# hzxie/Stereo-3D-Reconstruction

Hardware: AMD Instinct MI355X
Metric: stereo pairs/s forward (batch 32, 224x224 -> 32^3 voxel) (higher is better)
Workload: dtype f32

## Files before the change

include/s3r.h:

```cpp
#ifndef S3R_H
#define S3R_H

#include <stddef.h>
#include <stdint.h>

#ifdef __cplusplus
extern "C" {
#endif

#define S3R_ABI_VERSION 8

typedef enum s3r_status {
    S3R_OK = 0,
    S3R_ERR_INVALID = -1,
    S3R_ERR_HIP = -2,
    S3R_ERR_WORKSPACE = -3
} s3r_status;

typedef enum s3r_op {
    S3R_OP_CONV = 0,
    S3R_OP_DECONV = 1,
    S3R_OP_LINEAR = 2
} s3r_op;

typedef enum s3r_dtype {
    S3R_F32 = 0,
    S3R_BF16 = 1
} s3r_dtype;

typedef enum s3r_act { S3R_ACT_NONE = 0, S3R_ACT_RELU = 1, S3R_ACT_SIGMOID = 2,
                       S3R_ACT_LEAKY_RELU = 3, S3R_ACT_ELU = 4, S3R_ACT_TANH = 5  } s3r_act;

typedef enum s3r_layout { S3R_LAYOUT_PLAIN = 0, S3R_LAYOUT_WINO_H = 2, S3R_LAYOUT_WINO_DH = 3, S3R_LAYOUT_WINO_HW = 4,
                          S3R_LAYOUT_WINO_3D = 5, S3R_LAYOUT_DIFF = 6 } s3r_layout;

typedef enum s3r_algo { S3R_ALGO_AUTO = 0, S3R_ALGO_DIRECT = 1, S3R_ALGO_WINOGRAD = 2 } s3r_algo;

typedef struct s3r_conv_desc {
    int32_t op;
    int32_t ndim;
    int32_t batch;
    int32_t cin, cout;
    int32_t in_size;
    int32_t k, stride, pad;
    int32_t act;
    int32_t tag;
    int32_t tile;
    int32_t in_halo;
    int32_t out_halo;
    int32_t ksplit;
    int32_t dtype;
    int32_t in_layout;
    int32_t out_layout;
    int32_t algo;
    int32_t dilation;
    int32_t out_pad;
    float act_param;
} s3r_conv_desc;

typedef struct s3r_layer {
    s3r_conv_desc desc;
    const void* packed_w;
    const float* scale;
    const float* shift;
} s3r_layer;

int s3r_abi_version(void);
const char* s3r_last_error(void);

int s3r_conv_out_size(const s3r_conv_desc* d);
int s3r_conv_packed_elems(const s3r_conv_desc* d, int64_t* elems);
int s3r_conv_pack_weights(const s3r_conv_desc* d, const float* w, void* packed, void* stream);
int64_t s3r_conv_scratch_elems(const s3r_conv_desc* d);
int s3r_conv_forward(const s3r_conv_desc* d, const void* x, const void* packed_w, const float* scale,
                     const float* shift, void* y, float* scratch, int64_t scratch_elems, void* stream);

int64_t s3r_chain_workspace_elems(const s3r_layer* layers, int n_layers);
int s3r_chain_forward(const s3r_layer* layers, int n_layers, const void* x, void* y, float* ws, int64_t ws_elems,
                      int ws_fresh, void* stream);

int s3r_encoder_forward(const s3r_layer* layers, int n_layers, const float* images_left, const float* images_right,
                        void* features, float* ws, int64_t ws_elems, int ws_fresh, void* stream);
int s3r_decoder_forward(const s3r_layer* layers, int n_layers, const void* volume, float* occupancy, float* ws,
                        int64_t ws_elems, int ws_fresh, void* stream);

int s3r_encoder_forward_u8(const s3r_layer* layers, int n_layers, const uint8_t* images_left, const uint8_t* images_right,
                           void* features, float* ws, int64_t ws_elems, int ws_fresh, void* stream);

int s3r_channels_last_to_f32(const void* x, float* y, int batch, int channels, int64_t positions, void* stream);

int s3r_cost_volume_forward(const float* feat_left, const float* feat_right, float* volume, int batch, int channels,
                            int max_disp, int height, int width, int out_halo, void* stream);

int s3r_cost_volume_forward_wino(const float* feat_left, const float* feat_right, float* planes, int batch, int channels,
                                 int max_disp, int height, int width, void* stream);
int64_t s3r_conv_wino_input_elems(const s3r_conv_desc* d);
int s3r_conv_wino_input_layout(const s3r_conv_desc* d);
int s3r_cost_volume_forward_wino2(const float* feat_left, const float* feat_right, float* planes, int batch, int channels,
                                  int max_disp, int height, int width, void* stream);

int s3r_cost_volume_forward_bf16(const void* feat_left, const void* feat_right, void* volume, int batch, int channels,
                                 int max_disp, int height, int width, int out_halo, void* stream);

int s3r_cost_volume_backward(const float* grad_volume, float* grad_left, float* grad_right, int batch, int channels,
                             int max_disp, int height, int width, void* hip_stream);

int64_t s3r_linear_scratch_elems(int batch, int cin, int cout);
int s3r_linear_forward(const float* x, const float* w, const float* bias, float* y, int batch, int cin, int cout,
                       int act, float* scratch, int64_t scratch_elems, void* stream);

int64_t s3r_linear_backward_scratch_elems(int batch, int cin, int cout);
int s3r_linear_backward(const float* x, const float* w, const float* y, const float* grad_y, float* grad_x, float* grad_w,
                        float* grad_bias, int batch, int cin, int cout, int act, float* scratch, int64_t scratch_elems, void* stream);

int s3r_chamfer_forward(const float* p, const float* q, float* dist1, float* dist2, int32_t* idx1, int32_t* idx2,
                        int batch, int n, int m, void* stream);

int s3r_chamfer_backward(const float* p, const float* q, const int32_t* idx1, const int32_t* idx2, const float* grad_dist1,
                         const float* grad_dist2, float* grad_p, float* grad_q, int batch, int n, int m, void* stream);

int s3r_voxel_iou(const float* pred, const float* gt, float threshold, float* iou, int batch, int64_t voxels,
                  void* stream);

int s3r_voxel_bce_forward(const float* pred, const float* target, float* loss_sum, float* loss_elem, int batch, int64_t voxels,
                          void* stream);

int s3r_voxel_bce_backward(const float* pred, const float* target, const float* grad_scale, float* grad_pred, int batch,
                           int64_t voxels, void* stream);

int64_t s3r_head_backward_scratch_elems(int batch, int channels, int64_t voxels);
int s3r_head_backward(const float* x, const float* w, const float* scale, const float* y, const float* grad_y, float* grad_x,
                      float* grad_w, float* grad_shift, int batch, int channels, int64_t voxels, int act, float* scratch,
                      int64_t scratch_elems, void* stream);

#define S3R_CONV_BACKWARD_TAG 1000000
int s3r_conv_adjoint_desc(const s3r_conv_desc* d, s3r_conv_desc* adj);
int64_t s3r_conv_backward_scratch_elems(const s3r_conv_desc* d);
int s3r_conv_backward(const s3r_conv_desc* d, const float* x, const float* y, const float* grad_y, const float* scale, float* gs,
                      float* grad_w, float* grad_shift, float* scratch, int64_t scratch_elems, void* hip_stream);

int64_t s3r_batchnorm_train_forward_scratch_elems(int batch, int channels, int64_t positions);
int s3r_batchnorm_train_forward(const float* z, const float* gamma, const float* beta, float eps, int act, float* y, float* save_mean,
                                float* save_var, float* save_invstd, int batch, int channels, int64_t positions, float* scratch,
                                int64_t scratch_elems, void* hip_stream);
int64_t s3r_batchnorm_train_backward_scratch_elems(int batch, int channels, int64_t positions);
int s3r_batchnorm_train_backward(const float* z, const float* y, const float* grad_y, const float* gamma, const float* save_mean,
                                 const float* save_invstd, int act, float* grad_z, float* grad_gamma, float* grad_beta, int batch,
                                 int channels, int64_t positions, float* scratch, int64_t scratch_elems, void* hip_stream);

int s3r_disparity_wta(const float* feat_l, const float* feat_r, float* disp_l, float* disp_r, int batch, int channels,
                      int height, int width, int max_disp, void* stream);

// ... 31 lines not shown
```

stereo-3d-reconstruction_amd/_lib.py:

```python
from __future__ import annotations

import ctypes as C
import os
import threading

_HERE = os.path.dirname(os.path.abspath(__file__))
LIB_PATH = os.environ.get("S3R_LIB") or os.path.join(_HERE, "csrc", "libs3r_hip.so")

OP_CONV, OP_DECONV, OP_LINEAR = 0, 1, 2
DTYPE = {"fp32": 0, "bf16": 1}
ACT = {"none": 0, "relu": 1, "sigmoid": 2, "leaky_relu": 3, "elu": 4, "tanh": 5}
FAMILY = {0: "conv_mfma", 1: "stem", 2: "head", 3: "cost_volume", 4: "linear", 5: "chamfer", 6: "iou", 7: "pack",
          8: "pad_copy", 9: "disparity", 10: "aux"}
ABI_VERSION = 8
CONV_BACKWARD_TAG = 1000000
ALGO_AUTO, ALGO_DIRECT, ALGO_WINOGRAD = 0, 1, 2
ALGO = {None: 0, "auto": 0, "direct": 1, "winograd": 2, False: 1, True: 2}
RAN = {0: "direct", 1: "winograd-serial", 2: "winograd-class-parallel", 3: "winograd-dual", 4: "winograd-2axis", 5: "winograd-3axis", 6: "winograd-3axis-class-parallel"}


class ConvDesc(C.Structure):
    _fields_ = [(n, C.c_int32) for n in
                ("op", "ndim", "batch", "cin", "cout", "in_size", "k", "stride", "pad", "act", "tag", "tile",
                 "in_halo", "out_halo", "ksplit", "dtype", "in_layout", "out_layout", "algo", "dilation", "out_pad")] + \
               [("act_param", C.c_float)]


class Layer(C.Structure):
    _fields_ = [("desc", ConvDesc), ("packed_w", C.c_void_p), ("scale", C.c_void_p), ("shift", C.c_void_p)]


class ProfRecord(C.Structure):
    _fields_ = [("family", C.c_int32), ("tag", C.c_int32), ("ms", C.c_float), ("launches", C.c_int32),
                ("flops", C.c_double), ("bytes", C.c_double), ("exec_flops", C.c_double), ("algo", C.c_int32),
                ("reserved", C.c_int32)]


class S3RError(RuntimeError):
    pass


_lib = None
_lock = threading.Lock()

SIGNATURES = {
    "s3r_abi_version": (C.c_int, []),
    "s3r_last_error": (C.c_char_p, []),
    "s3r_conv_out_size": (C.c_int, [C.POINTER(ConvDesc)]),
    "s3r_conv_packed_elems": (C.c_int, [C.POINTER(ConvDesc), C.POINTER(C.c_int64)]),
    "s3r_conv_pack_weights": (C.c_int, [C.POINTER(ConvDesc), C.c_void_p, C.c_void_p, C.c_void_p]),
    "s3r_conv_scratch_elems": (C.c_int64, [C.POINTER(ConvDesc)]),
    "s3r_conv_forward": (C.c_int, [C.POINTER(ConvDesc), C.c_void_p, C.c_void_p, C.c_void_p, C.c_void_p, C.c_void_p,
                                   C.c_void_p, C.c_int64, C.c_void_p]),
    "s3r_chain_workspace_elems": (C.c_int64, [C.POINTER(Layer), C.c_int]),
    "s3r_chain_forward": (C.c_int, [C.POINTER(Layer), C.c_int, C.c_void_p, C.c_void_p, C.c_void_p, C.c_int64,
                                    C.c_int, C.c_void_p]),
    "s3r_encoder_forward": (C.c_int, [C.POINTER(Layer), C.c_int, C.c_void_p, C.c_void_p, C.c_void_p, C.c_void_p,
                                      C.c_int64, C.c_int, C.c_void_p]),
    "s3r_encoder_forward_u8": (C.c_int, [C.POINTER(Layer), C.c_int, C.c_void_p, C.c_void_p, C.c_void_p, C.c_void_p,
                                         C.c_int64, C.c_int, C.c_void_p]),
    "s3r_channels_last_to_f32": (C.c_int, [C.c_void_p, C.c_void_p, C.c_int, C.c_int, C.c_int64, C.c_void_p]),
    "s3r_decoder_forward": (C.c_int, [C.POINTER(Layer), C.c_int, C.c_void_p, C.c_void_p, C.c_void_p, C.c_int64,
                                      C.c_int, C.c_void_p]),
    "s3r_cost_volume_forward": (C.c_int, [C.c_void_p, C.c_void_p, C.c_void_p, C.c_int, C.c_int, C.c_int, C.c_int,
                                          C.c_int, C.c_int, C.c_void_p]),
    "s3r_cost_volume_forward_bf16": (C.c_int, [C.c_void_p, C.c_void_p, C.c_void_p, C.c_int, C.c_int, C.c_int, C.c_int,
                                               C.c_int, C.c_int, C.c_void_p]),
    "s3r_cost_volume_forward_wino": (C.c_int, [C.c_void_p, C.c_void_p, C.c_void_p, C.c_int, C.c_int, C.c_int, C.c_int,
                                               C.c_int, C.c_void_p]),
    "s3r_conv_wino_input_elems": (C.c_int64, [C.POINTER(ConvDesc)]),
    "s3r_conv_wino_input_layout": (C.c_int, [C.POINTER(ConvDesc)]),
    "s3r_cost_volume_forward_wino2": (C.c_int, [C.c_void_p, C.c_void_p, C.c_void_p, C.c_int, C.c_int, C.c_int, C.c_int,
                                                C.c_int, C.c_void_p]),
    "s3r_cost_volume_backward": (C.c_int, [C.c_void_p, C.c_void_p, C.c_void_p, C.c_int, C.c_int, C.c_int, C.c_int, C.c_int,
                                           C.c_void_p]),
    "s3r_linear_scratch_elems": (C.c_int64, [C.c_int, C.c_int, C.c_int]),
    "s3r_linear_forward": (C.c_int, [C.c_void_p, C.c_void_p, C.c_void_p, C.c_void_p, C.c_int, C.c_int, C.c_int,
                                     C.c_int, C.c_void_p, C.c_int64, C.c_void_p]),
    "s3r_linear_backward_scratch_elems": (C.c_int64, [C.c_int, C.c_int, C.c_int]),
    "s3r_linear_backward": (C.c_int, [C.c_void_p, C.c_void_p, C.c_void_p, C.c_void_p, C.c_void_p, C.c_void_p, C.c_void_p,
                                      C.c_int, C.c_int, C.c_int, C.c_int, C.c_void_p, C.c_int64, C.c_void_p]),
    "s3r_chamfer_forward": (C.c_int, [C.c_void_p, C.c_void_p, C.c_void_p, C.c_void_p, C.c_void_p, C.c_void_p,
                                      C.c_int, C.c_int, C.c_int, C.c_void_p]),
    "s3r_chamfer_backward": (C.c_int, [C.c_void_p, C.c_void_p, C.c_void_p, C.c_void_p, C.c_void_p, C.c_void_p, C.c_void_p, C.c_void_p,
                                       C.c_int, C.c_int, C.c_int, C.c_void_p]),
    "s3r_voxel_iou": (C.c_int, [C.c_void_p, C.c_void_p, C.c_float, C.c_void_p, C.c_int, C.c_int64, C.c_void_p]),
    "s3r_voxel_bce_forward": (C.c_int, [C.c_void_p, C.c_void_p, C.c_void_p, C.c_void_p, C.c_int, C.c_int64, C.c_void_p]),
    "s3r_voxel_bce_backward": (C.c_int, [C.c_void_p, C.c_void_p, C.c_void_p, C.c_void_p, C.c_int, C.c_int64, C.c_void_p]),
    "s3r_head_backward_scratch_elems": (C.c_int64, [C.c_int, C.c_int, C.c_int64]),
    "s3r_head_backward": (C.c_int, [C.c_void_p, C.c_void_p, C.c_void_p, C.c_void_p, C.c_void_p, C.c_void_p, C.c_void_p, C.c_void_p,
                                    C.c_int, C.c_int, C.c_int64, C.c_int, C.c_void_p, C.c_int64, C.c_void_p]),
    "s3r_batchnorm_train_forward_scratch_elems": (C.c_int64, [C.c_int, C.c_int, C.c_int64]),
    "s3r_batchnorm_train_forward": (C.c_int, [C.c_void_p, C.c_void_p, C.c_void_p, C.c_float, C.c_int, C.c_void_p, C.c_void_p, C.c_void_p,
                                              C.c_void_p, C.c_int, C.c_int, C.c_int64, C.c_void_p, C.c_int64, C.c_void_p]),
    "s3r_batchnorm_train_backward_scratch_elems": (C.c_int64, [C.c_int, C.c_int, C.c_int64]),
    "s3r_batchnorm_train_backward": (C.c_int, [C.c_void_p, C.c_void_p, C.c_void_p, C.c_void_p, C.c_void_p, C.c_void_p, C.c_int, C.c_void_p,
                                               C.c_void_p, C.c_void_p, C.c_int, C.c_int, C.c_int64, C.c_void_p, C.c_int64, C.c_void_p]),
    "s3r_conv_adjoint_desc": (C.c_int, [C.POINTER(ConvDesc), C.POINTER(ConvDesc)]),
    "s3r_conv_backward_scratch_elems": (C.c_int64, [C.POINTER(ConvDesc)]),
    "s3r_conv_backward": (C.c_int, [C.POINTER(ConvDesc), C.c_void_p, C.c_void_p, C.c_void_p, C.c_void_p, C.c_void_p, C.c_void_p, C.c_void_p,
                                    C.c_void_p, C.c_int64, C.c_void_p]),
    "s3r_disparity_wta": (C.c_int, [C.c_void_p, C.c_void_p, C.c_void_p, C.c_void_p, C.c_int, C.c_int, C.c_int, C.c_int,
                                    C.c_int, C.c_void_p]),
    "s3r_disparity_epe": (C.c_int, [C.c_void_p, C.c_void_p, C.c_void_p, C.c_void_p, C.c_int, C.c_int64, C.c_void_p]),
    "s3r_disparity_soft": (C.c_int, [C.c_void_p, C.c_void_p, C.c_int, C.c_void_p, C.c_void_p, C.c_void_p, C.c_void_p, C.c_int,
                                     C.c_int, C.c_int, C.c_int, C.c_int, C.c_float, C.c_int, C.c_int, C.c_float, C.c_void_p]),
    "s3r_disparity_metrics": (C.c_int, [C.c_void_p, C.c_void_p, C.c_void_p, C.c_void_p, C.c_int, C.c_int64, C.c_void_p]),
    "s3r_profile_enable": (C.c_int, [C.c_int]),
    "s3r_profile_reset": (C.c_int, []),
    "s3r_profile_detail": (C.c_int, [C.c_int]),
    "s3r_profile_read": (C.c_int, [C.POINTER(ProfRecord), C.c_int]),
}


def load():
    global _lib
    if _lib is not None:
        return _lib
    with _lock:
        if _lib is not None:
            return _lib
        if not os.path.exists(LIB_PATH):
            raise S3RError(
                f"HIP extension not built: {LIB_PATH} is missing. Run `python -c 'import __graft_entry__ as g; "
                f"g.build()'` (or `make -C stereo-3d-reconstruction_amd/csrc`). There is no CPU fallback.")
        try:
            lib = C.CDLL(LIB_PATH)
        except OSError as e:
            raise S3RError(f"cannot load {LIB_PATH}: {e}") from e
        for name, (res, args) in SIGNATURES.items():
            fn = getattr(lib, name)
            fn.restype, fn.argtypes = res, args
        if lib.s3r_abi_version() != ABI_VERSION:
            raise S3RError("libs3r_hip.so ABI version mismatch")
        _lib = lib
    return _lib


def check(rc, what=""):
    if rc < 0:
        msg = load().s3r_last_error().decode("utf-8", "replace")
        raise S3RError(f"{what}: {msg} (code {rc})")
    return rc


LAYOUT_PLAIN, LAYOUT_WINO_H, LAYOUT_WINO_DH, LAYOUT_WINO_HW, LAYOUT_WINO_3D, LAYOUT_DIFF = 0, 2, 3, 4, 5, 6


def make_desc(layer, batch, in_size, tag=0, tile=-1, in_halo=0, out_halo=0, ksplit=0, dtype=0, in_layout=0, out_layout=0,
              algo=0):
    from . import arch_spec as _spec
    op = {"conv2d": OP_CONV, "conv3d": OP_CONV, "deconv3d": OP_DECONV, "deconv2d": OP_DECONV, "linear": OP_LINEAR}[layer.op]
    nd = _spec.ndim(layer)
    return ConvDesc(op, nd, batch, layer.cin, layer.cout, in_size, layer.k, layer.s, layer.p, ACT[layer.act], tag,
                    tile, in_halo, out_halo, ksplit, dtype, in_layout, out_layout, algo, getattr(layer, "dil", 1),
                    getattr(layer, "opad", 0), _spec.act_param(layer))


def profile_enable(max_records):
    check(load().s3r_profile_enable(int(max_records)), "profile_enable")


def profile_detail(level):
    check(load().s3r_profile_detail(int(level)), "profile_detail")


def profile_reset():
    check(load().s3r_profile_reset(), "profile_reset")


def profile_read(max_records=4096):
    buf = (ProfRecord * max_records)()
    n = check(load().s3r_profile_read(buf, max_records), "profile_read")
    return [dict(family=FAMILY.get(r.family, str(r.family)), tag=r.tag, ms=r.ms, launches=r.launches, flops=r.flops,
                 bytes=r.bytes, exec_flops=r.exec_flops, ran=RAN.get(r.algo, str(r.algo))) for r in buf[:n]]
```

stereo-3d-reconstruction_amd/csrc/s3r_api.hip:

```cpp
#include "s3r_host.h"

#include <cmath>
#include <cstdlib>
#include <cstring>

using namespace s3rh;

namespace {

inline bool misaligned16(const void* p) { return ((uintptr_t)p & 15) != 0; }
int bf16_align_fail(const char* what, const void* p) {
    return fail(S3R_ERR_INVALID, "%s must be 16-byte aligned (got %p): bf16 tensors are accessed 16 bytes at a time", what, p);
}

int wino2_run(const s3r_conv_desc* d, const Geo& g, s3r::ConvParams p, const float* x, const float* packed_w, float* y, float* scratch,
              int64_t scratch_elems, int form, hipStream_t s, int* launches) {
    const Wino2Geo g2 = wino2_geo(d);
    const WinoNeed need = wino2_need(d, form);
    const bool pre = d->in_layout == S3R_LAYOUT_WINO_DH || d->in_layout == S3R_LAYOUT_WINO_HW ||
                     d->in_layout == S3R_LAYOUT_WINO_3D;
    const bool to_v = d->out_layout == S3R_LAYOUT_WINO_HW;
    p.out_mode = d->out_layout == S3R_LAYOUT_WINO_3D ? (d->out_halo ? 1 : 2) : d->out_layout == S3R_LAYOUT_DIFF ? 3 : 0;
    if (p.out_mode && (g2.ax > 1 || wino2_form_of(d, (int)(g2.pos_sample * d->batch), form) != 0))
        return fail(S3R_ERR_INVALID, "a consumer's operand is written from the class-parallel launch form of a 3D two-axis layer only (the semi-fused "
                    "form of this batch keeps the plain output: s3r_chain_forward plans that itself)");
    if (g2.bmax <= 0 || ((pre || to_v || p.out_mode) && g2.bmax < d->batch))
        return fail(S3R_ERR_INVALID, "two-axis Winograd form: the transformed input of this batch exceeds 2 GiB (at most %d samples per "
                    "call with a producer-written input: s3r_conv_wino_input_elems)", g2.bmax);
    if (!scratch || scratch_elems < need.total)
        return fail(S3R_ERR_WORKSPACE, "the two-axis Winograd form of this layer needs %lld floats of scratch (s3r_conv_scratch_elems), "
                    "got %lld", (long long)need.total, (long long)(scratch ? scratch_elems : 0));
    const int64_t direct_w = ipow(d->k, g.nd) * d->cin * cout_pad(d->cout);
    p.w = packed_w + direct_w + (wino_layer(d) ? wino_w_elems(d) : 0);
    p.x = pre ? x : scratch;
    p.part = scratch + need.v;
    p.Nd = g2.sg; p.Nh = g2.sg; p.Nw = g2.out;
    p.kd = 1; p.kh = 1; p.kw = g2.kw; p.T = g2.kw;
    p.x_hs = g2.wp; p.x_ds = g2.sg * g2.wp; p.x_cs = g2.sg * g2.sg * g2.wp;
    p.x_org = 0;
    p.dS = s3r::FastDiv((unsigned)(p.Nd * p.Nh * p.Nw));
    p.dHW = s3r::FastDiv((unsigned)(p.Nh * p.Nw));
    p.dW = s3r::FastDiv((unsigned)p.Nw);
    if (g2.ax == 2) {
        p.Nd = 1; p.Nw = g2.sg;
        p.dS = s3r::FastDiv((unsigned)(g2.sg * g2.sg));
        p.dW = s3r::FastDiv((unsigned)g2.sg);
    }
    p.Hout = g2.out; p.Dout = g2.out;
    p.ncls = g2.ncls;
    p.ksplit = 1;
    const int64_t x_sample = g.x_elems / d->batch;
    *launches = 0;
    for (int b0 = 0; b0 < d->batch; b0 += g2.bmax) {
        const int nb = d->batch - b0 < g2.bmax ? d->batch - b0 : g2.bmax;
        hipError_t e = hipSuccess;
        if (!pre) {
            s3r::AuxScope aux(s, 4.0 * ((double)nb * x_sample + (double)(g2.ax == 2 ? g2.ncls * d->cin * s3r::wino2_npad(g2.pos_sample * nb) : g2.v_sample * nb)));
            if (g2.ax == 2)
                e = s3r::launch_wino2p_input(x + (int64_t)b0 * x_sample, scratch, nb, d->cin, g2.wp, g2.wp, g2.sg, g2.sg,
                                             s3r::wino2_npad(g2.pos_sample * nb), s);
            else
                e = s3r::launch_wino2_input(x + (int64_t)b0 * x_sample, scratch, g2.ax, (long long)nb * d->cin, g2.wp, g2.wp, g2.wp, g2.sg, g2.sg, s);
            if (e != hipSuccess) return hip_fail(e, "two-axis Winograd input transform launch");
            *launches += 1;
        }
        p.B = nb;
        p.x_cls = nb * d->cin * p.x_cs;
        p.x_bytes = (unsigned)(4 * (int64_t)nb * g2.v_sample);
        p.Ntotal = nb * p.Nd * p.Nh * p.Nw;
        p.y = y + (int64_t)b0 * p.y_bs;
        p.y_bytes = (unsigned)(4 * (int64_t)nb * p.y_bs);
        int nl = 0;
        e = s3r::launch_conv_wino2(p, g2.ax, wino2_form_of(d, p.Ntotal, form), to_v, s, &nl);
// ... 1191 lines not shown
```

stereo-3d-reconstruction_amd/csrc/s3r_conv_wino.hip:

```cpp
#include "s3r_kernels.h"
#include <cstdlib>

namespace s3r {

typedef float wf32x16 __attribute__((ext_vector_type(16)));
typedef float wv2f __attribute__((ext_vector_type(2)));
template <int N> struct WVec;
template <> struct WVec<1> { typedef float type; };
template <> struct WVec<2> { typedef wv2f type; };
typedef float wv4f __attribute__((ext_vector_type(4)));
template <> struct WVec<4> { typedef wv4f type; };
template <int N>
__device__ __forceinline__ float wvget(const typename WVec<N>::type& v, int i) {
    if constexpr (N == 1) return v; else return v[i];
}

#define S3R_LDS_PTR_W(p) ((__attribute__((address_space(3))) void*)(p))

#ifndef S3R_WNB
#define S3R_WNB 2
#endif
#ifndef S3R_WBK
#define S3R_WBK 32
#endif
constexpr int WBM = 64, WBK = S3R_WBK, WNB = S3R_WNB;
constexpr int WNPA = WBK * WBM / 1024;
int wino_bk() { return WBK; }

#ifdef S3R_ABLATE
__device__ unsigned long long s3r_wino_timeline[6 * 65536];
#endif

template <int BYTES>
__device__ __forceinline__ void wdma(__amdgpu_buffer_rsrc_t rsrc, float* lds_dst, int voffset, int soffset) {
    static_assert(BYTES == 16 || BYTES == 4, "LDS-DMA width");
    if constexpr (BYTES == 16) __builtin_amdgcn_raw_ptr_buffer_load_lds(rsrc, S3R_LDS_PTR_W(lds_dst), 16, voffset, soffset, 0, 0);
    else __builtin_amdgcn_raw_ptr_buffer_load_lds(rsrc, S3R_LDS_PTR_W(lds_dst), 4, voffset, soffset, 0, 0);
}

template <int R>
__global__ __launch_bounds__(256) void wino_input_kernel(const float* __restrict__ x, float* __restrict__ V, long long planes,
                                                         int Hp, int Wp, int Hq, long long cls_stride) {
    const long long total = planes * Hq * Wp;
    for (long long i = (long long)blockIdx.x * 256 + threadIdx.x; i < total; i += (long long)gridDim.x * 256) {
        const long long row = i / Wp;
        const int w = (int)(i - row * Wp);
        const long long pl = row / Hq;
        const int q = (int)(row - pl * Hq);
        const float* __restrict__ src = x + (pl * Hp + R * q) * Wp + w;
        float r[R + 2], v[R + 2];
#pragma unroll
        for (int k = 0; k < R + 2; ++k) r[k] = (R * q + k < Hp) ? src[(long long)k * Wp] : 0.f;
        wino_rows_to_classes<R>(r, v);
#pragma unroll
// ... 130 lines not shown
            const int kw = 3 - rw - 2 * tw;
            const float* g = w + ((size_t)cin * Cout + co) * 64 + kw;
            auto hsum = [&](int td) {
                const float* gd = g + (3 - rd - 2 * td) * 16;
                const float g0 = gd[(3 - rh) * 4], g1 = gd[(1 - rh) * 4];
                return fb == 0 ? g0 : fb == 2 ? g1 : g0 + g1;
            };
            v = fa == 0 ? hsum(0) : fa == 2 ? hsum(1) : hsum(0) + hsum(1);
        }
        wp[i] = v;
    }
}

hipError_t launch_pack_wino_deconv(const float* w, float* wp, int Cin, int Cout, int CoutPad, hipStream_t s) {
    hipLaunchKernelGGL(pack_wino_deconv_kernel, dim3(1024), dim3(256), 0, s, w, wp, Cin, Cout, CoutPad);
    return hipGetLastError();
}

template <int KIND> struct WinoKind;
template <> struct WinoKind<1> { static constexpr int NCLS = 6, R = 4; };
template <> struct WinoKind<2> { static constexpr int NCLS = 9, R = 4; };

template <int KIND>
__device__ __forceinline__ void wino_out(const float (&m)[WinoKind<KIND>::NCLS], float (&y)[WinoKind<KIND>::R]) {
    if constexpr (KIND == 1) {
        const float s12 = m[1] + m[2], d12 = m[1] - m[2];
        const float s34 = m[3] + m[4], d34 = m[3] - m[4];
        y[0] = (m[0] + s12) + s34;
        y[1] = fmaf(2.f, d34, d12);
        y[2] = fmaf(4.f, s34, s12);
        y[3] = fmaf(8.f, d34, d12) + m[5];
    } else {
        const float t00 = m[0] + m[1], t01 = m[1] - m[2];
        const float t10 = m[3] + m[4], t11 = m[4] - m[5];
        const float t20 = m[6] + m[7], t21 = m[7] - m[8];
        y[0] = t00 + t10;
        y[1] = t01 + t11;
        y[2] = t10 - t20;
        y[3] = t11 - t21;
    }
}
template <int KIND>
__device__ __forceinline__ int wino_out_off(int i, int y_ds, int y_hs) {
    if constexpr (KIND == 1) return i * y_hs;
    else return (i >> 1) * 2 * y_ds + (i & 1) * 2 * y_hs;
}
__device__ __forceinline__ float wino_act(float y, float sc, float sf, float lo) { return fmaxf(fmaf(y, sc, sf), lo); }
__device__ __forceinline__ float wino_head_act(float t, int act) {
    if (act == ACT_RELU) return fmaxf(t, 0.f);
    if (act == ACT_SIGMOID) return __builtin_amdgcn_rcpf(1.f + __expf(-t));
    return t;
}

template <int VEC, int KIND, int WN, bool CP, bool HEAD, bool XM = false, bool SEMI = false>
__device__ __forceinline__ void wino_body(const ConvParams& p, const int bid_in, const int nwg_in, const int n_begin,
                                          const int n_end, float* __restrict__ wsmem) {
    constexpr bool DECONV = KIND == 2;
    constexpr int NCLS = WinoKind<KIND>::NCLS, R = WinoKind<KIND>::R;
    constexpr int WM = 4 / WN, TM = 2 / WM, BN = 32 * WN;
    constexpr int NACC = CP ? 1 : NCLS;
    static_assert(KIND == 1 || KIND == 2, "F(4,3) convolution or F(2,2) transposed convolution");
    static_assert(!SEMI || (KIND == 1 && !CP && !HEAD), "the semi-fused form: serial F(4,3) row classes of one depth class");
    static_assert(WN == 4 || WN == 2, "4 waves as 1 x 4 or 2 x 2");
    static_assert(!HEAD || (DECONV && !CP && WN == 2), "the fused head: serial transposed form");
    float* As = wsmem;
    constexpr int BSTG = (DECONV ? 2 : 1) * WBK * BN;
    float* Bs = wsmem + WNB * WBK * WBM;
    constexpr int PB = 64 * VEC;
    constexpr int NPIECE_B = WBK * BN / PB;
    static_assert(NPIECE_B % 4 == 0, "B pieces divide over the 4 waves");
    constexpr int NPB = NPIECE_B / 4;
    constexpr bool B_WIDE = BN >= PB;
    constexpr int PPR = B_WIDE ? BN / PB : 1;
    constexpr int RPP = B_WIDE ? 1 : PB / BN;
    constexpr int LPR_B = BN / VEC;
    constexpr int NPD = WNPA + NPB;

    const int tid = threadIdx.x;
    const int lane = tid & 63;
    const int wave = __builtin_amdgcn_readfirstlane(tid >> 6);
    const int wm = wave / WN, wn = wave % WN;
    const int j = lane & 31, h = lane >> 5;
#ifdef S3R_ABLATE
    unsigned long long tl0 = 0, tl1 = 0, tl2 = 0;
    if (p.debug == 7) tl0 = __builtin_amdgcn_s_memrealtime();
#endif

    const int n_tiles = (n_end - n_begin + BN - 1) / BN;
    int bid = bid_in, cls0 = 0, pc = 0;
    if constexpr (CP || SEMI) {
        const int nwg = nwg_in;
        const int q = nwg >> 3, r = nwg & 7, xcd = bid & 7, slot = bid >> 3;
        const int item = (xcd < r ? xcd * (q + 1) : r * (q + 1) + (xcd - r) * q) + slot;
        const int ntile = p.m_tiles * n_tiles;
        const int c = item / ntile;
        bid = item - c * ntile;
        if constexpr (DECONV) { pc = c / NCLS; cls0 = c - pc * NCLS; } else cls0 = SEMI ? c * NCLS : c;
    } else if constexpr (DECONV) {
        const int nwg = nwg_in >> 3;
        const int item = (bid & 7) * nwg + (bid >> 3);
        bid = item >> 3;
        pc = item & 7;
    } else {
        const int nwg = nwg_in;
        const int q = nwg >> 3, r = nwg & 7, xcd = bid & 7, slot = bid >> 3;
        bid = (xcd < r ? xcd * (q + 1) : r * (q + 1) + (xcd - r) * q) + slot;
    }
    const int rd = (pc >> 2) & 1, rh = (pc >> 1) & 1, rw = pc & 1;
    const int m_tile = bid % p.m_tiles, n_tile = bid / p.m_tiles;
    const int m0 = m_tile * WBM, n0 = n_begin + n_tile * BN;
    const int S = p.Nd * p.Nh * p.Nw;
    const int T = DECONV ? 2 : p.T;
    const int chunks = p.Cin / WBK;
    const int nkt = T * chunks;
    const int total = NACC * nkt;

    int bvoff;
    {
        int col, lrow;
        if (B_WIDE) { col = (wave % PPR) * PB + lane * VEC; lrow = 0; }
        else        { col = (lane % LPR_B) * VEC;           lrow = lane / LPR_B; }
        int n = n0 + col;
        if (n >= n_end) n = n_end - VEC;
        const int b = p.dS.div(n);
        int rem = n - b * S;
        const int pd = p.dHW.div(rem);
        rem -= pd * p.Nh * p.Nw;
        const int q = p.dW.div(rem);
        const int pw = rem - q * p.Nw;
        if constexpr (DECONV)
            bvoff = (b * p.Cin * p.x_cs + (2 * pd + rd) * p.x_ds + (2 * q + rh) * p.x_hs + pw + rw + lrow * p.x_cs) * 4;
        else
            bvoff = (b * p.Cin * p.x_cs + p.x_org + pd * p.x_ds + q * p.x_hs + pw + lrow * p.x_cs) * 4;
    }
    const int avoff = ((lane >> 4) * p.CoutPad + (lane & 15) * 4) * 4;
    const __amdgpu_buffer_rsrc_t xrsrc =
        __builtin_amdgcn_make_buffer_rsrc(const_cast<float*>(p.x), 0, (int)p.x_bytes, 0x00020000);
    const __amdgpu_buffer_rsrc_t drsrc =
        __builtin_amdgcn_make_buffer_rsrc(const_cast<float*>(DECONV ? p.xd : p.x), 0, (int)p.x_bytes, 0x00020000);
    const size_t x_el = (size_t)p.x_bytes / 4;
    const __amdgpu_buffer_rsrc_t wrsrc = __builtin_amdgcn_make_buffer_rsrc(
        const_cast<float*>(p.w), 0,
        (int)((unsigned)(DECONV ? 72 : (p.ncls ? p.ncls : NCLS)) * (unsigned)T * (unsigned)p.Cin * (unsigned)p.CoutPad * 4u),
        0x00020000);
    const int b_row0 = B_WIDE ? wave / PPR : wave * RPP;
    constexpr int B_ROW_STEP = B_WIDE ? 4 / PPR : 4 * RPP;
    const int b_lds0 = B_WIDE ? b_row0 * BN + (wave % PPR) * PB : wave * PB;
    constexpr int B_LDS_STEP = B_WIDE ? B_ROW_STEP * BN : 4 * PB;
    const int cs4 = p.x_cs * 4;

    int c_cls = cls0, c_cc = 0, c_td = 0, c_tw = 0, c_tap = 0;
    int c_kt = (DECONV ? pc * NCLS + cls0 : cls0) * nkt;
    int c_a = cls0 / 3, c_b = cls0 - 3 * (cls0 / 3);
#ifdef S3R_ABLATE
    bool abl_loop = false;
#endif
    auto issue = [&](int buf) __attribute__((always_inline)) {
#ifdef S3R_ABLATE
        const bool skip_a = abl_loop && (p.debug == 3 || p.debug == 5);
        const bool skip_b = abl_loop && (p.debug == 3 || p.debug == 4 || (p.debug == 6 && (DECONV ? c_tap != 0 : c_tw != 0)));
#else
        constexpr bool skip_a = false, skip_b = false;
#endif
        if (!skip_a) {
#pragma unroll
            for (int q = 0; q < WNPA; ++q)
                wdma<16>(wrsrc, As + buf * WBK * WBM + (wave + 4 * q) * 256, avoff,
                         (c_kt * WBK * p.CoutPad + m0) * 4 + (wave + 4 * q) * 4 * p.CoutPad * 4);
        }
        float* sb = Bs + buf * BSTG + b_lds0;
        if constexpr (DECONV) {
            const int b_base = ((c_cc * WBK + b_row0) * p.x_cs + (c_a ? p.x_ds : 0) + (c_b ? p.x_hs : 0) + c_tap) * 4;
            if (skip_b) {
            } else if constexpr (XM) {
                const int t_idx = (c_a != 1 ? 2 : 0) + (c_b != 1 ? 1 : 0);
                const float* tb = t_idx == 0 ? p.x : p.xd + (size_t)(t_idx - 1) * x_el;
                const __amdgpu_buffer_rsrc_t trsrc = __builtin_amdgcn_make_buffer_rsrc(const_cast<float*>(tb), 0, (int)p.x_bytes, 0x00020000);
#pragma unroll
                for (int q = 0; q < NPB; ++q) wdma<4 * VEC>(trsrc, sb + q * B_LDS_STEP, bvoff, b_base + q * B_ROW_STEP * cs4);
            } else if (c_b == 1) {
#pragma unroll
                for (int q = 0; q < NPB; ++q) wdma<4 * VEC>(xrsrc, sb + q * B_LDS_STEP, bvoff, b_base + q * B_ROW_STEP * cs4);
                if (c_a != 1) {
#pragma unroll
                    for (int q = 0; q < NPB; ++q)
                        wdma<4 * VEC>(xrsrc, sb + WBK * BN + q * B_LDS_STEP, bvoff, b_base + p.x_ds * 4 + q * B_ROW_STEP * cs4);
                }
            } else {
#pragma unroll
                for (int q = 0; q < NPB; ++q) wdma<4 * VEC>(drsrc, sb + q * B_LDS_STEP, bvoff, b_base + q * B_ROW_STEP * cs4);
                if (c_a != 1) {
#pragma unroll
                    for (int q = 0; q < NPB; ++q)
                        wdma<4 * VEC>(drsrc, sb + WBK * BN + q * B_LDS_STEP, bvoff, b_base + p.x_ds * 4 + q * B_ROW_STEP * cs4);
                }
            }
            ++c_kt;
            if (++c_tap == 2) {
                c_tap = 0;
                if (++c_cc == chunks) {
                    c_cc = 0; ++c_cls;
                    if (++c_b == 3) { c_b = 0; ++c_a; }
                }
            }
        } else {
            const int b_base = (c_cls * p.x_cls + (c_cc * WBK + b_row0) * p.x_cs + c_td * p.x_ds + c_tw) * 4;
            if (!skip_b) {
#pragma unroll
                for (int q = 0; q < NPB; ++q) wdma<4 * VEC>(xrsrc, sb + q * B_LDS_STEP, bvoff, b_base + q * B_ROW_STEP * cs4);
            }
            ++c_kt;
            if (++c_tw == p.kw) { c_tw = 0; ++c_td; }
            if (++c_tap == T) {
                c_tap = 0; c_td = 0; c_tw = 0;
                if (++c_cc == chunks) { c_cc = 0; ++c_cls; }
            }
        }
    };

    wf32x16 acc[NACC][TM];
#pragma unroll
    for (int c = 0; c < NACC; ++c)
#pragma unroll
        for (int t = 0; t < TM; ++t)
#pragma unroll
            for (int r = 0; r < 16; ++r) acc[c][t][r] = 0.f;

#pragma unroll
    for (int i = 0; i < WNB - 1; ++i)
        if (i < total) issue(i);
    if (total >= WNB - 1) asm volatile("s_waitcnt vmcnt(%0)" :: "n"((WNB - 2) * NPD) : "memory");
    else asm volatile("s_waitcnt vmcnt(0)" ::: "memory");
    __builtin_amdgcn_s_barrier();
    asm volatile("" ::: "memory");
#ifdef S3R_ABLATE
    abl_loop = true;
    if (p.debug == 7) tl1 = __builtin_amdgcn_s_memrealtime();
#endif

    const int a_off = h * WBM + wm * TM * 32 + j * TM;
    const int b_off = h * BN + wn * 32 + j;
    typedef typename WVec<TM>::type AV;
    int cur = 0, g = 0;
    auto run_class = [&](wf32x16 (&ac)[TM], const bool diff) __attribute__((always_inline)) {
        for (int kt = 0; kt < nkt; ++kt, ++g) {
            const bool more = g + WNB - 1 < total;
            if (more) issue(cur == 0 ? WNB - 1 : cur - 1);
            const float* a = As + cur * WBK * WBM + a_off;
            const float* b = Bs + cur * BSTG + b_off;
            if (DECONV && diff) {
#pragma unroll
                for (int ks = 0; ks < WBK / 2; ++ks) {
                    const AV av = *reinterpret_cast<const AV*>(a + ks * 2 * WBM);
                    const float bv = b[ks * 2 * BN] - b[WBK * BN + ks * 2 * BN];
#pragma unroll
                    for (int t = 0; t < TM; ++t) ac[t] = __builtin_amdgcn_mfma_f32_32x32x2f32(wvget<TM>(av, t), bv, ac[t], 0, 0, 0);
                }
            } else {
#pragma unroll
                for (int ks = 0; ks < WBK / 2; ++ks) {
                    const AV av = *reinterpret_cast<const AV*>(a + ks * 2 * WBM);
                    const float bv = b[ks * 2 * BN];
#pragma unroll
                    for (int t = 0; t < TM; ++t) ac[t] = __builtin_amdgcn_mfma_f32_32x32x2f32(wvget<TM>(av, t), bv, ac[t], 0, 0, 0);
                }
            }
            if (more) asm volatile("s_waitcnt vmcnt(%0)" :: "n"((WNB - 2) * NPD) : "memory");
            else asm volatile("s_waitcnt vmcnt(0)" ::: "memory");
// ... 123 lines not shown
                t0 = fmaf(wino_act(y[0], sc, sf, lo), hw, t0);
                t1 = fmaf(wino_act(y[1], sc, sf, lo), hw, t1);
                t2 = fmaf(wino_act(y[2], sc, sf, lo), hw, t2);
                t3 = fmaf(wino_act(y[3], sc, sf, lo), hw, t3);
                if ((r & 3) == 3) __builtin_amdgcn_sched_barrier(0);
            }
            t0 += __shfl_xor(t0, 32, 64);
            t1 += __shfl_xor(t1, 32, 64);
            t2 += __shfl_xor(t2, 32, 64);
            t3 += __shfl_xor(t3, 32, 64);
            float* ex = wsmem + 4 * WBM + (wn * 32 + j) * 4;
            if (wm == 1 && h == 0) { ex[0] = t0; ex[1] = t1; ex[2] = t2; ex[3] = t3; }
            __syncthreads();
            if (wm == 0 && h == 0 && ok) {
                const float hsc = p.head_scale ? p.head_scale[0] : 1.f, hsf = p.head_shift ? p.head_shift[0] : 0.f;
                p.y[e0] = wino_head_act(fmaf(t0 + ex[0], hsc, hsf), p.head_act);
                p.y[e0 + wino_out_off<KIND>(1, p.y_ds, p.y_hs)] = wino_head_act(fmaf(t1 + ex[1], hsc, hsf), p.head_act);
                p.y[e0 + wino_out_off<KIND>(2, p.y_ds, p.y_hs)] = wino_head_act(fmaf(t2 + ex[2], hsc, hsf), p.head_act);
                p.y[e0 + wino_out_off<KIND>(3, p.y_ds, p.y_hs)] = wino_head_act(fmaf(t3 + ex[3], hsc, hsf), p.head_act);
            }
        } else {
            const __amdgpu_buffer_rsrc_t yrsrc = __builtin_amdgcn_make_buffer_rsrc(p.y, 0, (int)p.y_bytes, 0x00020000);
            const int yvo0 = (e0 + (m0 + mbase) * p.y_cs) * 4;
            const int row_bytes = p.y_cs * 4;
#pragma unroll
            for (int tm = 0; tm < TM; ++tm)
#pragma unroll
                for (int r = 0; r < 16; ++r) {
                    const int dm = ((r & 3) + 8 * (r >> 2)) * TM + tm;
                    if (dm >= mlimit) continue;
                    const float sc = ep_sc[mbase + dm], sf = ep_sf[mbase + dm];
                    float m[NCLS], y[R];
#pragma unroll
                    for (int c = 0; c < NCLS; ++c) m[c] = acc[c][tm][r];
                    wino_out<KIND>(m, y);
                    const int so = dm * row_bytes;
                    if (ok) {
#pragma unroll
                        for (int i = 0; i < R; ++i)
                            if (i < row1) {
                                const float v = wino_act(y[i], sc, sf, lo);
                                __builtin_amdgcn_raw_buffer_store_b32(__builtin_bit_cast(unsigned, v), yrsrc,
                                                                      yvo0 + 4 * wino_out_off<KIND>(i, p.y_ds, p.y_hs), so, 0);
                            }
                    }
                    if ((r & 3) == 3) __builtin_amdgcn_sched_barrier(0);
                }
        }
        S3R_TL_FINISH();
    }
}
#undef S3R_TL_FINISH

template <int VEC, int KIND, int WN, bool CP, bool HEAD, bool XM = false, bool SEMI = false>
__global__ __launch_bounds__(256, (CP || KIND == 1 ? 4 : 3)) void wino_kernel(const ConvParams p) {
    extern __shared__ __attribute__((aligned(16))) float wsmem[];
    wino_body<VEC, KIND, WN, CP, HEAD, XM, SEMI>(p, blockIdx.x, gridDim.x, p.n_begin, p.n_end, wsmem);
}

template <int VEC, int KIND, bool HEAD = false, bool XM = false>
__global__ __launch_bounds__(256, (KIND == 1 ? 4 : 3)) void wino_dual_kernel(const ConvParams p) {
    extern __shared__ __attribute__((aligned(16))) float wsmem[];
    if ((int)blockIdx.x < p.big_wgs)
        wino_body<VEC, KIND, 2, false, HEAD, XM>(p, blockIdx.x, p.big_wgs, p.n_begin, p.n_cut, wsmem);
    else
        wino_body<VEC, KIND, 2, true, false, XM>(p, (int)blockIdx.x - p.big_wgs, (int)gridDim.x - p.big_wgs, p.n_cut, p.n_end, wsmem);
}

template <int KIND, bool HEAD>
__global__ __launch_bounds__(256) void wino_finish_kernel(const ConvParams p, const int n_begin, const int n_end, const int npad) {
    constexpr bool DECONV = KIND == 2;
    constexpr int NCLS = WinoKind<KIND>::NCLS, R = WinoKind<KIND>::R;
    const int S = p.Nd * p.Nh * p.Nw;
    const int nn = n_end - n_begin;
    const int pc = DECONV ? (int)blockIdx.y : 0;
    const int rd = (pc >> 2) & 1, rh = (pc >> 1) & 1, rw = pc & 1;
    const float lo = p.act == ACT_RELU ? 0.f : -__builtin_inff();
    constexpr int NBLK = DECONV ? 8 * NCLS : NCLS;
    const int ntl = npad >> 6;
    const float* __restrict__ base = p.part + (size_t)pc * NCLS * 64;
    auto blk = [&](int mm, int nl) { return base + ((size_t)mm * ntl + (nl >> 6)) * (NBLK * 64) + (nl & 63); };
    const long long total = HEAD ? nn : (long long)p.Cout * nn;
    for (long long i = (long long)blockIdx.x * 256 + threadIdx.x; i < total; i += (long long)gridDim.x * 256) {
        const int mrow = HEAD ? 0 : (int)(i / nn);
        const int nl = (int)(i - (long long)mrow * nn);
        const int n = n_begin + nl;
        const int b = p.dS.div(n);
        int rem = n - b * S;
        const int pd = p.dHW.div(rem);
        rem -= pd * p.Nh * p.Nw;
        const int q = p.dW.div(rem);
        const int pw = rem - q * p.Nw;
        int e0, row1 = R;
        if constexpr (DECONV)
            e0 = b * p.y_bs + p.y_org + (2 * pd * p.y_ds + 2 * q * p.y_hs + pw) * 2 + rd * p.y_ds + rh * p.y_hs + rw;
        else {
            e0 = b * p.y_bs + p.y_org + pd * p.y_ds + R * q * p.y_hs + pw;
            row1 = p.Hout - R * q;
        }
        if constexpr (HEAD) {
            float tw[2][R];
#pragma unroll
            for (int wm = 0; wm < 2; ++wm) {
                float th[2][R];
#pragma unroll
                for (int hh = 0; hh < 2; ++hh) {
#pragma unroll
                    for (int k = 0; k < R; ++k) th[hh][k] = 0.f;
                    for (int r = 0; r < 16; ++r) {
                        const int mm = 32 * wm + 4 * hh + (r & 3) + 8 * (r >> 2);
// ... 286 lines not shown
                for (int kh = 0; kh < R; ++kh) gh[kh] = g[(kd * R + kh) * R];
                gd[kd] = wax_g<AX>(cb, gh);
            }
            v = wax_g<AX>(ca, gd);
        }
        wp[i] = v;
    }
}

__global__ void pack_wino2p_kernel(const float* __restrict__ w, float* __restrict__ wp, int Cin, int Cout, int CoutPad);
hipError_t launch_pack_wino2(const float* w, float* wp, int ax, int Cin, int Cout, int CoutPad, hipStream_t s) {
    if (ax == 0) hipLaunchKernelGGL(pack_wino2_kernel<0>, dim3(1024), dim3(256), 0, s, w, wp, Cin, Cout, CoutPad);
    else if (ax == 1) hipLaunchKernelGGL(pack_wino2_kernel<1>, dim3(1024), dim3(256), 0, s, w, wp, Cin, Cout, CoutPad);
    else if (ax == 2) hipLaunchKernelGGL(pack_wino2p_kernel, dim3(1024), dim3(256), 0, s, w, wp, Cin, Cout, CoutPad);
    else return hipErrorInvalidValue;
    return hipGetLastError();
}

__device__ __forceinline__ void wino2_copy_out(const float* __restrict__ lds, float* __restrict__ dst, int count, int tid) {
    if ((count & 3) == 0 && (reinterpret_cast<size_t>(dst) & 15) == 0) {
        for (int i = tid * 4; i < count; i += 1024) *reinterpret_cast<wv4f*>(dst + i) = *reinterpret_cast<const wv4f*>(lds + i);
    } else {
        for (int i = tid; i < count; i += 256) dst[i] = lds[i];
    }
}
__device__ __forceinline__ void wino2_zero_out(float* __restrict__ dst, int count, int tid) {
    if ((count & 3) == 0 && (reinterpret_cast<size_t>(dst) & 15) == 0) {
        for (int i = tid * 4; i < count; i += 1024) *reinterpret_cast<wv4f*>(dst + i) = wv4f{0.f, 0.f, 0.f, 0.f};
    } else {
        for (int i = tid; i < count; i += 256) dst[i] = 0.f;
    }
}

__global__ __launch_bounds__(256) void wino2s_finish_kernel(const ConvParams p, const int npad, const int halo, const int SUB,
                                                            const FastDiv dNd, const FastDiv dMS) {
    constexpr int N = 6, M = 4;
    extern __shared__ __attribute__((aligned(16))) float fsm[];
    const int tid = threadIdx.x;
    const int G = p.Nh * p.Nw, Wp = p.y_hs, slice = p.y_ds, MS = M * slice;
    const float lo = p.act == ACT_RELU ? 0.f : -__builtin_inff();
    const int per_c = p.B * p.Nd;
    const int nrg = (per_c + SUB - 1) / SUB;
    const bool vec = (slice & 3) == 0 && (reinterpret_cast<size_t>(p.y) & 15) == 0;
    for (int item = blockIdx.x; item < p.Cout * nrg; item += gridDim.x) {
        const int mrow = item / nrg;
        const int r0 = (item - mrow * nrg) * SUB;
        const int nsub = per_c - r0 < SUB ? per_c - r0 : SUB;
        for (int i = tid; i < nsub * MS; i += 256) fsm[i] = 0.f;
        __syncthreads();
        const float sc = p.scale ? p.scale[mrow] : 1.f, sf = p.shift ? p.shift[mrow] : 0.f;
        for (int t = tid; t < nsub * G; t += 256) {
            const int sub = p.dHW.div(t);
            const int g = t - sub * G;
            const int sh = p.dW.div(g);
            const int pw = g - sh * p.Nw;
            const int r = r0 + sub;
            const int sd = r - dNd.div(r) * p.Nd;
            const int n = r0 * G + t;
            const float* __restrict__ src = p.part + ((size_t)mrow * (npad >> 6) + (n >> 6)) * (N * M * 64) + (n & 63);
            float* __restrict__ o = fsm + sub * MS + (halo + M * sh) * Wp + halo + pw;
#pragma unroll
            for (int v = 0; v < M; ++v) {
                float m[N], y[M];
#pragma unroll
                for (int a = 0; a < N; ++a) m[a] = src[(a * M + v) * 64];
                wax_at<0>(m, y);
#pragma unroll
                for (int u = 0; u < M; ++u)
                    if (M * sd + u < p.Dout && M * sh + v < p.Hout) o[u * slice + v * Wp] = wino_act(y[u], sc, sf, lo);
            }
        }
        __syncthreads();
        float* __restrict__ yc = p.y + (size_t)mrow * p.y_cs;
        for (int e = vec ? tid * 4 : tid; e < nsub * MS; e += vec ? 1024 : 256) {
            const int sub = dMS.div(e);
            const int off = e - sub * MS;
            const int r = r0 + sub;
            const int b = dNd.div(r);
            const int sd = r - b * p.Nd;
            const int nsl = p.Dout - M * sd < M ? p.Dout - M * sd : M;
            if (off >= nsl * slice) continue;
            float* __restrict__ dst = yc + (size_t)b * p.y_bs + (size_t)(halo + M * sd) * slice + off;
            if (vec) *reinterpret_cast<wv4f*>(dst) = *reinterpret_cast<const wv4f*>(fsm + e);
            else *dst = fsm[e];
        }
        if (halo > 0)
            for (int sub = 0; sub < nsub; ++sub) {
                const int r = r0 + sub;
                const int b = dNd.div(r);
                const int sd = r - b * p.Nd;
                if (sd == 0) wino2_zero_out(yc + (size_t)b * p.y_bs, halo * slice, tid);
                if (sd == p.Nd - 1) wino2_zero_out(yc + (size_t)b * p.y_bs + (size_t)(halo + p.Dout) * slice, halo * slice, tid);
            }
        __syncthreads();
    }
}

template <int AX>
__global__ __launch_bounds__(256) void wino2_finish_flat_kernel(const ConvParams p, const int npad) {
    constexpr int N = WAxis<AX>::N, M = WAxis<AX>::M;
    const int S = p.Nd * p.Nh * p.Nw;
    const int nn = p.Ntotal;
    const float lo = p.act == ACT_RELU ? 0.f : -__builtin_inff();
    const long long total = (long long)p.Cout * nn;
    for (long long i = (long long)blockIdx.x * 256 + threadIdx.x; i < total; i += (long long)gridDim.x * 256) {
        const int mrow = (int)(i / nn);
        const int n = (int)(i - (long long)mrow * nn);
        const int b = p.dS.div(n);
        int rem = n - b * S;
        const int sd = p.dHW.div(rem);
        rem -= sd * p.Nh * p.Nw;
        const int sh = p.dW.div(rem);
        const int pw = rem - sh * p.Nw;
        const float* __restrict__ src = p.part + ((size_t)mrow * (npad >> 6) + (n >> 6)) * (N * N * 64) + (n & 63);
        float t[N][M];
#pragma unroll
        for (int a = 0; a < N; ++a) {
            float m[N], y[M];
#pragma unroll
            for (int c = 0; c < N; ++c) m[c] = src[(a * N + c) * 64];
            wax_at<AX>(m, y);
#pragma unroll
            for (int v = 0; v < M; ++v) t[a][v] = y[v];
        }
        const float sc = p.scale ? p.scale[mrow] : 1.f, sf = p.shift ? p.shift[mrow] : 0.f;
        float* __restrict__ yo = p.y + (size_t)b * p.y_bs + (size_t)mrow * p.y_cs + p.y_org + (size_t)M * sd * p.y_ds + M * sh * p.y_hs + pw;
#pragma unroll
        for (int v = 0; v < M; ++v) {
            float m[N], y[M];
#pragma unroll
            for (int a = 0; a < N; ++a) m[a] = t[a][v];
            wax_at<AX>(m, y);
#pragma unroll
            for (int u = 0; u < M; ++u)
                if (M * sd + u < p.Dout && M * sh + v < p.Hout) yo[(size_t)u * p.y_ds + v * p.y_hs] = wino_act(y[u], sc, sf, lo);
        }
    }
}

__global__ __launch_bounds__(256) void wino2p_input_kernel(const float* __restrict__ x, float* __restrict__ V, unsigned total, int Cin,
                                                           int Hp, int Wp, int SH, int SW, unsigned npad, unsigned nn, FastDiv dSW,
                                                           FastDiv dSH, FastDiv dN) {
    constexpr int N = 6, M = 4;
    const size_t cstride = (size_t)Cin * npad;
    for (unsigned i = blockIdx.x * 256u + threadIdx.x; i < total; i += gridDim.x * 256u) {
        const unsigned c = (unsigned)dN.div((int)i);
        const unsigned n = i - c * nn;
        const unsigned row = (unsigned)dSW.div((int)n);
        const int sw = (int)(n - row * (unsigned)SW);
        const unsigned b = (unsigned)dSH.div((int)row);
        const int sh = (int)(row - b * (unsigned)SH);
        const float* __restrict__ src = x + (((size_t)b * Cin + c) * Hp + M * sh) * Wp + M * sw;
        float t[N][N];
#pragma unroll
        for (int jc = 0; jc < N; ++jc) {
            float r[N], v[N];
#pragma unroll
            for (int ir = 0; ir < N; ++ir) r[ir] = (M * sh + ir < Hp && M * sw + jc < Wp) ? src[(size_t)ir * Wp + jc] : 0.f;
            wax_bt<0>(r, v);
#pragma unroll
            for (int ir = 0; ir < N; ++ir) t[ir][jc] = v[ir];
        }
        float* __restrict__ dst = V + (size_t)c * npad + n;
#pragma unroll
        for (int bb = 0; bb < N; ++bb) {
            float v[N];
// ... 355 lines not shown
    if ((cons == 0 && (halo != 1 || On < 4)) || (cons == 1 && (halo != 0 || On < 5)) || (cons == 2 && (halo != 1 || (On & 3)))) return hipErrorInvalidValue;
    const int SG = cons == 0 ? (On + 3) / 4 : cons == 1 ? (On - 2) / 2 : 1;
    const int vol = Op * Op * Op;
    if (vol > 8192) return hipErrorInvalidValue;
    const int CB = 8192 / vol < 8 ? 8192 / vol : 8;
    const int S = p.Nd * p.Nh * p.Nw;
    if (p.Ntotal != p.B * S || npad < p.Ntotal) return hipErrorInvalidValue;
    double slabs;
    if (prod <= 1) {
        if (p.ncls != wino2_classes(prod) || p.Dout != On || p.Hout != On || p.Nw != On || p.act == ACT_SIGMOID) return hipErrorInvalidValue;
        slabs = (double)p.ncls * npad;
    } else if (prod == 2) {
        if (!p.transposed || cons != 2 || 2 * p.Nw != On || 4 * p.Nd != On || 4 * p.Nh != On || p.act == ACT_SIGMOID) return hipErrorInvalidValue;
        slabs = 72.0 * npad;
    } else {
        if (p.transposed || cons == 2 || p.ksplit <= 1 || p.y_step > 1 || p.shuf_s || p.Nd != On || p.Nh != On || p.Nw != On || p.act == ACT_SIGMOID)
            return hipErrorInvalidValue;
        slabs = (double)p.ksplit * npad;
    }
    const int G1 = prod == 2 ? 8 * S : S, G2 = cons == 2 ? vol : SG * SG * Op;
    const double written = cons == 2 ? 4.0 * p.B * vol : (double)wino2_classes(cons) * p.B * G2;
    if ((double)p.Cout * written >= 2147483648.0) return hipErrorInvalidValue;
    const long long items = (long long)p.B * ((p.Cout + CB - 1) / CB);
    const dim3 grid((unsigned)(items < 16384 ? items : 16384));
    const size_t lds = (size_t)CB * vol * sizeof(float);
    const FastDiv dG1((unsigned)G1), dG2((unsigned)G2), dOp((unsigned)Op), dOp2((unsigned)(Op * Op)), dSG((unsigned)SG);
    AuxScope aux(stream, 4.0 * (double)p.Cout * (slabs + written));
#define S3R_HANDOFF(PR, CO) hipLaunchKernelGGL((wino_handoff_kernel<PR, CO>), grid, dim3(256), lds, stream, p, npad, CB, On, halo, SG, dG1, dG2, dOp, dOp2, dSG)
    switch (prod * 3 + cons) {
        case 0: S3R_HANDOFF(0, 0); break;
        case 1: S3R_HANDOFF(0, 1); break;
        case 2: S3R_HANDOFF(0, 2); break;
        case 3: S3R_HANDOFF(1, 0); break;
        case 4: S3R_HANDOFF(1, 1); break;
        case 5: S3R_HANDOFF(1, 2); break;
        case 8: S3R_HANDOFF(2, 2); break;
        case 9: S3R_HANDOFF(3, 0); break;
        case 10: S3R_HANDOFF(3, 1); break;
        default: return hipErrorInvalidValue;
    }
#undef S3R_HANDOFF
    return hipGetLastError();
}

int wino2_form(int ax, int cout, int ntotal, int forced) {
    if (ax == 1) return 0;
    if (forced >= 0) return forced ? 1 : 0;
    static const int env_form = getenv("S3R_WINO2_FORM") ? atoi(getenv("S3R_WINO2_FORM")) : -1;
    if (env_form >= 0) return env_form ? 1 : 0;
    const long semi_wgs = (long)((cout + WBM - 1) / WBM) * ((ntotal + WCN - 1) / WCN) * 6;
    return semi_wgs >= (ax == 2 ? 2 : 8) * (long)cu_count() ? 1 : 0;
}
int64_t wino2_npad(int64_t ntotal) { return (ntotal + WCN - 1) / WCN * WCN; }
int64_t wino2_slab_elems(int ax, int cout, int ntotal, int form) {
    const int64_t npad = (int64_t)((ntotal + WCN - 1) / WCN) * WCN;
    return (form ? 6 * 4 : wino2_classes(ax)) * (int64_t)cout * npad;
}

hipError_t launch_conv_wino2(ConvParams p, int ax, int form, bool to_v, hipStream_t stream, int* launches) {
    if (p.Cin % WBK != 0 || p.stride != 1 || p.transposed || p.ksplit != 1 || p.head_w || p.act == ACT_SIGMOID || !p.part ||
        ax < 0 || ax > 2 || p.ncls != wino2_classes(ax))
        return hipErrorInvalidValue;
    p.kh = 1;
    S3R_WABL(p);
    p.m_tiles = (p.Cout + WBM - 1) / WBM;
    p.n_begin = 0; p.n_end = p.Ntotal;
    const int n_tiles = (p.Ntotal + WCN - 1) / WCN;
    const size_t lds = (size_t)WNB * WBK * (WBM + WCN) * sizeof(float);
    const int halo = to_v ? 1 : (p.y_hs - p.Hout) / 2;
    if (to_v && (ax != 2 || p.Hout % 4 != 0)) return hipErrorInvalidValue;
    if (p.out_mode && (to_v || ax == 2 || form != 0)) return hipErrorInvalidValue;
    if (!to_v && (halo < 0 || p.y_hs != p.Hout + 2 * halo)) return hipErrorInvalidValue;
    if (ax == 2) {
        const int plane = to_v ? (p.Hout + 2) * (p.Hout + 2) : p.y_hs * p.y_hs, G = p.Nh * p.Nw;
        if ((!to_v && p.y_cs != plane) || (size_t)plane * 4 > 64 * 1024) return hipErrorInvalidValue;
        int PL = 256 / G < 1 ? 1 : 256 / G;
        if (PL > p.B) PL = p.B;
        while (PL > 1 && (size_t)PL * plane * 4 > 64 * 1024) --PL;
        const int npad = n_tiles * WCN;
        ConvParams q = p;
        q.B = 1; q.Nd = 1; q.Nh = 1; q.Nw = npad;
        q.dS = q.dHW = q.dW = FastDiv((unsigned)npad);
        q.kd = q.kh = q.kw = 1; q.T = 1;
        q.x_org = 0; q.x_ds = 0; q.x_hs = 0; q.x_cs = npad; q.x_cls = p.Cin * npad;
        q.x_bytes = (unsigned)(4ull * 36 * p.Cin * npad);
        q.Ntotal = npad; q.n_end = npad;
        const dim3 grid(p.m_tiles * n_tiles * (form == 1 ? 6 : 36));
        if (form == 1) hipLaunchKernelGGL((wino_kernel<4, 1, 2, false, false, false, true>), grid, dim3(256), lds, stream, q);
        else hipLaunchKernelGGL((wino_kernel<4, 1, 2, true, false>), grid, dim3(256), lds, stream, q);
        hipError_t e = hipGetLastError();
        if (e != hipSuccess) return e;
        const long long items = (long long)p.Cout * ((p.B + PL - 1) / PL);
        const dim3 fgrid((unsigned)(items < 16384 ? items : 16384));
        const size_t flds = (size_t)PL * plane * 4;
        AuxScope aux(stream, 4.0 * (double)p.Cout * ((double)(form == 1 ? 24 : 36) * npad + (to_v ? 36.0 * npad : (double)p.B * plane)));
        if (to_v) {
            if (form == 1) hipLaunchKernelGGL((wino2p_finish_kernel<true, true>), fgrid, dim3(256), flds, stream, p, npad, halo, PL);
            else hipLaunchKernelGGL((wino2p_finish_kernel<false, true>), fgrid, dim3(256), flds, stream, p, npad, halo, PL);
        } else if (form == 1) hipLaunchKernelGGL((wino2p_finish_kernel<true, false>), fgrid, dim3(256), flds, stream, p, npad, halo, PL);
        else hipLaunchKernelGGL((wino2p_finish_kernel<false, false>), fgrid, dim3(256), flds, stream, p, npad, halo, PL);
        if (launches) *launches = 2;
        return hipGetLastError();
    }
    if (p.y_ds != p.y_hs * p.y_hs || p.y_cs != (p.Dout + 2 * halo) * p.y_ds) return hipErrorInvalidValue;
    if (form == 1) {
        const int M = wino2_outputs(ax), G = p.Nh * p.Nw;
        if (ax != 0 || (size_t)M * p.y_ds * 4 > 64 * 1024) return hipErrorInvalidValue;
        int SUB = 256 / G < 1 ? 1 : 256 / G;
        if (SUB > p.B * p.Nd) SUB = p.B * p.Nd;
        while (SUB > 1 && (size_t)SUB * M * p.y_ds * 4 > 64 * 1024) --SUB;
        const size_t flds = (size_t)SUB * M * p.y_ds * 4;
        const FastDiv dNd((unsigned)p.Nd), dMS((unsigned)(M * p.y_ds));
        const long long items = (long long)p.Cout * ((p.B * p.Nd + SUB - 1) / SUB);
        const dim3 fgrid((unsigned)(items < 32768 ? items : 32768));
        const dim3 grid(p.m_tiles * n_tiles * 6);
        if (p.Nw % 4 == 0) hipLaunchKernelGGL((wino_kernel<4, 1, 2, false, false, false, true>), grid, dim3(256), lds, stream, p);
        else hipLaunchKernelGGL((wino_kernel<1, 1, 2, false, false, false, true>), grid, dim3(256), lds, stream, p);
        hipError_t e = hipGetLastError();
        if (e != hipSuccess) return e;
        AuxScope aux(stream, 4.0 * (double)p.Cout * (24.0 * n_tiles * WCN + (double)p.B * p.y_cs));
        hipLaunchKernelGGL(wino2s_finish_kernel, fgrid, dim3(256), flds, stream, p, n_tiles * WCN, halo, SUB, dNd, dMS);
        if (launches) *launches = 2;
        return hipGetLastError();
    }
    const dim3 grid(p.m_tiles * n_tiles * p.ncls);
    if (p.Nw % 4 == 0) hipLaunchKernelGGL((wino_kernel<4, 1, 2, true, false>), grid, dim3(256), lds, stream, p);
    else hipLaunchKernelGGL((wino_kernel<1, 1, 2, true, false>), grid, dim3(256), lds, stream, p);
    hipError_t e = hipGetLastError();
    if (e != hipSuccess) return e;
    if (launches) *launches = 2;
    if (p.out_mode) return launch_wino_handoff(p, ax, p.out_mode - 1, n_tiles * WCN, stream);
    const long long total = (long long)p.Cout * p.Ntotal;
    const long long blocks = (total + 255) / 256;
    const dim3 flat((unsigned)(blocks < 8192 ? blocks : 8192));
    AuxScope aux(stream, 4.0 * (double)p.Cout * ((double)p.ncls * n_tiles * WCN + (double)p.B * p.Dout * p.Hout * p.Nw));
    if (ax == 0) hipLaunchKernelGGL(wino2_finish_flat_kernel<0>, flat, dim3(256), 0, stream, p, n_tiles * WCN);
    else hipLaunchKernelGGL(wino2_finish_flat_kernel<1>, flat, dim3(256), 0, stream, p, n_tiles * WCN);
    if (launches) *launches = 2;
    return hipGetLastError();
}

#ifdef S3R_ABLATE
}
extern "C" int s3r_debug_read_timeline_wino(unsigned long long* out, int nblocks) {
    if (nblocks > 65536) nblocks = 65536;
    return hipMemcpyFromSymbol(out, HIP_SYMBOL(s3r::s3r_wino_timeline), sizeof(unsigned long long) * 6 * (size_t)nblocks) == hipSuccess ? nblocks : -1;
}
extern "C" int s3r_debug_clear_timeline_wino() {
    void* ptr = nullptr;
    if (hipGetSymbolAddress(&ptr, HIP_SYMBOL(s3r::s3r_wino_timeline)) != hipSuccess) return -1;
    return hipMemset(ptr, 0, sizeof(unsigned long long) * 6 * 65536) == hipSuccess ? 0 : -1;
}
namespace s3r {
#endif

}
```

stereo-3d-reconstruction_amd/csrc/s3r_host.h:

```cpp
#pragma once
#include "../../include/s3r.h"
#include "s3r_kernels.h"

#include <cstdint>
#include <vector>

namespace s3rh {

constexpr int64_t kMaxElems = (int64_t)1 << 31;
constexpr int64_t kMaxBytes = (int64_t)1 << 32;

const char* last_error();

enum Family { F_MFMA = 0, F_STEM = 1, F_HEAD = 2, F_COSTVOL = 3, F_LINEAR = 4, F_CHAMFER = 5, F_IOU = 6, F_PACK = 7, F_PAD = 8, F_DISP = 9,
              F_AUX = 10 };

struct ProfScope {
    bool active = false;
    int slot = -1;
    unsigned gen = 0;
    hipEvent_t e0 = nullptr, e1 = nullptr;
    int launches = 1;
    int algo = 0;
    double exec = -1.0;
// ... 50 lines not shown
int out_size(const s3r_conv_desc* d);
int dil_of(const s3r_conv_desc* d);
bool staged_layer(const s3r_conv_desc* d);
struct StagedGeo { int cin_pad, step, pe, sp; int64_t elems; int bmax; };
StagedGeo staged_geo(const s3r_conv_desc* d);
s3r::ConvParams make_params_staged(const s3r_conv_desc* d, const Geo& g);
struct TClassAxis { int kr, ke, qmin, nq; };
bool im2col_layer(const s3r_conv_desc* d);
bool leaky_fused(const s3r_conv_desc* d);
bool needs_act_pass(const s3r_conv_desc* d);
bool tclass_layer(const s3r_conv_desc* d);
bool tclass_direct(const s3r_conv_desc* d);
bool tshuf_layer(const s3r_conv_desc* d);
s3r::ConvParams make_params_tshuf(const s3r_conv_desc* d, const Geo& g);
int want_halo(const s3r_conv_desc* d, Route r);
TClassAxis tclass_axis(const s3r_conv_desc* d, int r);
int tclass_halo(const s3r_conv_desc* d);
int64_t tclass_w_elems(const s3r_conv_desc* d);
bool make_params_tclass(const s3r_conv_desc* d, const Geo& g, int rd, int rh, int rw, s3r::ConvParams* q, int64_t* w_off, double* macs);
int geometry(const s3r_conv_desc* d, Geo* g);
int route(const s3r_conv_desc* d, Route* r);
int need_halo(const s3r_conv_desc* d, Route r);
int check_halos(const s3r_conv_desc* d, Route r);
int cout_pad(int cout);
int wino_mode();
bool wino_layer(const s3r_conv_desc* d);
bool dwino_layer(const s3r_conv_desc* d);
bool dwino3_layer(const s3r_conv_desc* d);
bool dwino3_desc_ok(const s3r_conv_desc* d);
int64_t dwino3_w_offset(const s3r_conv_desc* d);
struct Dwino3Need { int64_t diff, total; bool split; };
Dwino3Need dwino3_need(const s3r_conv_desc* d, int form);
bool wino_desc_ok(const s3r_conv_desc* d);
int wino2_ax(const s3r_conv_desc* d);
bool wino2_desc_ok(const s3r_conv_desc* d);
int wino2_max_edge();
int resolve_algo(const s3r_conv_desc* d, int* alg, int* form);
bool resolves_to_wino(const s3r_conv_desc* d);
Wino2Geo wino2_geo(const s3r_conv_desc* d);
int64_t wino_w_elems(const s3r_conv_desc* d);
int64_t wino_v_elems(const s3r_conv_desc* d);
int wino_bmax(const s3r_conv_desc* d);
int64_t dwino_w_elems(const s3r_conv_desc* d);
bool dwino_materialise(const s3r_conv_desc* d);
int64_t dwino_d_elems(const s3r_conv_desc* d);
int wino_kind(const s3r_conv_desc* d);
int wino_kcls(const s3r_conv_desc* d);
int64_t wino_positions(const s3r_conv_desc* d, int nb);
WinoNeed wino_need(const s3r_conv_desc* d, int form, bool head);
double wino_exec_flops(const s3r_conv_desc* d, const Geo& g);
int wino2_form_of(const s3r_conv_desc* d, int ntotal, int forced);
WinoNeed wino2_need(const s3r_conv_desc* d, int form);
double wino2_exec_flops(const s3r_conv_desc* d);
int cout_pad_h(int cout);
s3r::ConvParamsH make_params_h(const s3r_conv_desc* d, const Geo& g);
int resolve_launch_h(const s3r_conv_desc* d, s3r::ConvParamsH* p, LaunchH* L);
s3r::ConvParams make_params(const s3r_conv_desc* d, const Geo& g);
int resolve_launch(const s3r_conv_desc* d, s3r::ConvParams* p, Launch* L);
int64_t align_up(int64_t v, int64_t a);
int plan_chain(const s3r_layer* layers, int n, Plan* pl);

}
```

stereo-3d-reconstruction_amd/csrc/s3r_kernels.h:

```cpp
#pragma once
#include <hip/hip_runtime.h>
#include <stdint.h>
#include <atomic>

namespace s3r {

struct LdsAttr {
    std::atomic<unsigned long long> done{0};
    hipError_t ensure(const void* fn, int bytes) {
        int dev = 0;
        hipError_t e = hipGetDevice(&dev);
        if (e != hipSuccess) return e;
        if (dev >= 0 && dev < 64 && ((done.load(std::memory_order_relaxed) >> dev) & 1ull)) return hipSuccess;
        e = hipFuncSetAttribute(fn, hipFuncAttributeMaxDynamicSharedMemorySize, bytes);
        if (e == hipSuccess && dev >= 0 && dev < 64) done.fetch_or(1ull << dev, std::memory_order_relaxed);
        return e;
    }
};

inline int cu_count() {
    static std::atomic<int> cached[64];
    int dev = 0;
    if (hipGetDevice(&dev) != hipSuccess || dev < 0) { (void)hipGetLastError(); return 256; }
    int n = dev < 64 ? cached[dev].load(std::memory_order_relaxed) : 0;
// ... 25 lines not shown
#endif
};

#if defined(__HIPCC__)
__device__ __forceinline__ float render_f32(float v) { return v; }
__device__ __forceinline__ float render_f32(unsigned char u) {
    const float f = (float)u;
    const float rcp = 1.f / 255.f;
    const float q = __fmul_rn(f, rcp);
    return fmaf(fmaf(-q, 255.f, f), rcp, q);
}
#endif

struct ConvParams {
    const float* x;
    const float* w;
    const float* scale;
    const float* shift;
    float* y;
    int B, Cin, Cout, CoutPad;
    int Nd, Nh, Nw;
    FastDiv dS, dHW, dW;
    int kd, kh, kw, T;
    int stride;
    int dil;
    int x_cs, x_ds, x_hs;
    int x_org;
    int y_cs, y_ds, y_hs;
    int y_bs;
    int y_org;
    int y_step;
    int shuf_s, shuf_nd;
    FastDiv dSC, dS1;
    unsigned x_bytes;
    unsigned y_bytes;
    int transposed;
    int act;
    float slope;
    int Ntotal;
    int n_begin, n_end;
    int n_tiles, m_tiles;
    int n_cut, big_wgs;
    int ksplit;
    float* part;
    int debug;
    const float* head_w;
    const float* head_scale;
    const float* head_shift;
    int head_act;
    int x_cls, Hout, Dout, ncls;
    const float* xd;
    int xd_mode;
    int out_mode;
};

struct TClsEntry {
    int Nd, Nh, Nw, kd, kh, kw, T, x_org, y_org, Ntotal, wg_begin, w_off;
    FastDiv dS, dHW, dW;
};
constexpr int kTClsMax = 27;
struct TClsTable { int n; TClsEntry e[kTClsMax]; };
hipError_t launch_conv_tcls(const ConvParams& base, TClsTable tab, hipStream_t stream);

enum { WINO_SERIAL = 0, WINO_CP = 1, WINO_DUAL = 2 };
struct WinoLaunch { int mode, n_cut; };

struct ConvParamsH {
    const void* x;
    const void* w;
    const float* scale;
    const float* shift;
    void* y;
    float* part;
    int B, Cin, Cout, CoutPad;
    int Nd, Nh, Nw;
    FastDiv dS, dHW, dW, dDH, dH;
    int kd, kh, kw, T;
    int stride;
    int x_bs, x_ds, x_hs, x_ws;
    int x_org;
    int y_bs, y_ds, y_hs, y_ws;
    int y_org;
    unsigned x_bytes;
    int transposed, act, Ntotal;
    int m_tiles, n_tiles;
    int ksplit;
    int debug;
    const float* head_w;
    const float* head_scale;
    const float* head_shift;
    int head_act;
};

enum { ACT_NONE = 0, ACT_RELU = 1, ACT_SIGMOID = 2 };

hipError_t launch_conv_mfma(const ConvParams& p, int tile_code, hipStream_t stream);
int conv_pick_tile(const ConvParams& p);
int conv_pick_vec(const ConvParams& p);
int conv_pick_ksplit(const ConvParams& p, int tile_cfg);
int64_t conv_scratch_elems(const ConvParams& p, int tile_cfg);
int conv_num_tiles();
int conv_last_launch_count();
void conv_tile_dims(int tile_cfg, int* bm, int* bn);
hipError_t launch_pack_conv(const float* w, float* wp, int Cin, int Cout, int CoutPad, int T, int transposed,
                            hipStream_t s);
hipError_t launch_wino_input(const float* x, float* V, long long planes, int Hp, int Wp, int Hq, int R, hipStream_t s);
hipError_t launch_pack_wino(const float* w, float* wp, int Cin, int Cout, int CoutPad, int kd, int kw, int R, hipStream_t s);
WinoLaunch wino_plan(int kind, int cout, int kcls, int ntotal, bool head, int forced);
int64_t wino_slab_elems(int kind, int cout, int ntotal, const WinoLaunch& L);
hipError_t launch_conv_wino(ConvParams p, const WinoLaunch& L, hipStream_t stream, int* launches);
int wino2_classes(int ax);
int wino2_outputs(int ax);
hipError_t launch_wino2_input(const float* x, float* V, int ax, long long planes, int Dp, int Hp, int Wp, int SD, int SH, hipStream_t s);
hipError_t launch_wino2p_input(const float* x, float* V, int B, int Cin, int Hp, int Wp, int SH, int SW, long long npad, hipStream_t s);
hipError_t launch_pack_wino2(const float* w, float* wp, int ax, int Cin, int Cout, int CoutPad, hipStream_t s);
int wino2_form(int ax, int cout, int ntotal, int forced);
int64_t wino2_slab_elems(int ax, int cout, int ntotal, int form);
int64_t wino2_npad(int64_t ntotal);
hipError_t launch_conv_wino2(ConvParams p, int ax, int form, bool to_v, hipStream_t stream, int* launches);
hipError_t launch_wino_handoff(const ConvParams& p, int prod, int cons, int npad, hipStream_t stream);
hipError_t launch_cost_volume_wino2(const float* fl, const float* fr, float* V, int B, int C, int D, int H, int W, hipStream_t s);
int wino_bk();
hipError_t launch_wino_diff(const float* x, float* D, long long planes, int Dp, int Hp, int Wp, int three, hipStream_t s);
hipError_t launch_pack_wino_deconv(const float* w, float* wp, int Cin, int Cout, int CoutPad, hipStream_t s);
hipError_t launch_deconv_wino(ConvParams p, const WinoLaunch& L, hipStream_t stream, int* launches);
hipError_t launch_pack_dwino3(const float* w, float* wp, int Cin, int Cout, hipStream_t s);
int64_t dwino3_w_elems(int Cin, int Cout);
bool dwino3_edge_ok(int n);
int64_t dwino3_slab_elems(int cout, int ntotal);
bool dwino3_split(int cout, int ntotal, int forced);
hipError_t launch_deconv_wino3(ConvParams p, bool split, hipStream_t stream);
hipError_t launch_stem_wino(const void* x, const void* x2, int u8, int nsplit, const float* wt, const float* scale, const float* shift,
                            float* V, int N, int Hi, int Wi, int Ho, int Wo, hipStream_t s);
hipError_t launch_stem(const void* x, const void* x2, int u8, int nsplit, const float* w, const float* scale,
                       const float* shift, float* y, int N, int Hi, int Wi, int Ho, int Wo, int y_cs, int y_hs, int y_org,
                       hipStream_t s);
hipError_t launch_cost_volume(const float* fl, const float* fr, float* vol, int B, int C, int D, int H, int W,
                              int halo, hipStream_t s);
hipError_t launch_cost_volume_wino(const float* fl, const float* fr, float* V, int B, int C, int D, int H, int W, int R, hipStream_t s);
hipError_t launch_zero_fill(float* y, long long n, hipStream_t s);
hipError_t launch_stage(const float* x, float* y, int B, int Cin, int CinPad, int nd, int n, int in_halo, int sp, int pe, int step,
                        hipStream_t s);
hipError_t launch_pack_general(const float* w, float* wp, int Cin, int CinPad, int Cout, int CoutPad, int T, int flip, hipStream_t s);
hipError_t launch_stage_im2col(const float* x, float* y, int B, int Cin, int KPad, int nd, int n, int in_halo, int n_out, int k, int stride,
                               int pad, int dil, hipStream_t s);
hipError_t launch_pack_tclass(const float* w, float* wp, int Cin, int CinPad, int Cout, int CoutPad, int nd, int k, int stride,
                              int rd, int rh, int rw, hipStream_t s);
hipError_t launch_act(float* y, long long total, int act, float param, hipStream_t s);
hipError_t launch_pad_copy(const float* x, float* y, int64_t planes, int D, int H, int W, int hd, int hh, int hw,
                           hipStream_t s);
hipError_t launch_pack_stem(const float* w, float* wt, hipStream_t s);
hipError_t launch_head(const float* x, const float* w, const float* scale, const float* shift, float* y, int B, int C,
                       int64_t S, int act, hipStream_t s);
hipError_t launch_chamfer(const float* p, const float* q, float* d1, float* d2, int* i1, int* i2,
                          int B, int N, int M, hipStream_t s);
hipError_t launch_chamfer_backward(const float* p, const float* q, const int* i1, const int* i2, const float* g1, const float* g2,
                                   float* gp, float* gq, int B, int N, int M, hipStream_t s);
hipError_t launch_linear(const float* x, const float* w, const float* scale, const float* bias, float* y, int B,
                         int Cin, int Cout, int act, float* scratch, hipStream_t s);
int64_t linear_scratch_elems(int B, int Cin, int Cout);
hipError_t launch_linear_backward(const float* x, const float* w, const float* y, const float* gy, float* gx, float* gw, float* gb,
                                  int B, int Cin, int Cout, int act, float* scratch, hipStream_t s, int* launches);
int64_t linear_backward_scratch_elems(int B, int Cin, int Cout);
hipError_t launch_head_backward(const float* x, const float* w, const float* scale, const float* y, const float* gy, float* gx,
                                float* gw, float* gshift, int B, int C, int64_t S, int act, float* scratch, hipStream_t s,
                                int* launches);
int64_t head_backward_scratch_elems(int B, int C, int64_t S);
hipError_t launch_batchnorm_train_forward(const float* z, const float* gamma, const float* beta, float eps, int act, float* y,
                                          float* mean, float* var, float* invstd, int B, int C, int64_t S, float* scratch, hipStream_t s,
// ... 72 lines not shown
```

stereo-3d-reconstruction_amd/csrc/s3r_plan.hip:

```cpp
#include "s3r_host.h"

#include <cstdarg>
#include <cstdio>
#include <cstdlib>
#include <cstring>

namespace s3rh {

thread_local char g_err[512] = "";

int fail(int code, const char* fmt, ...) {
    va_list ap;
    va_start(ap, fmt);
    vsnprintf(g_err, sizeof(g_err), fmt, ap);
    va_end(ap);
    return code;
}

int hip_fail(hipError_t e, const char* what) {
    return fail(S3R_ERR_HIP, "%s: %s", what, hipGetErrorString(e));
}

int64_t ipow(int64_t b, int e) {
    int64_t r = 1;
// ... 59 lines not shown
    return h;
}
bool tshuf_layer(const s3r_conv_desc* d) {
    return tclass_layer(d) && d->k == d->stride && d->stride >= 2 && d->pad == 0 && d->out_pad == 0;
}
int64_t tclass_w_elems(const s3r_conv_desc* d) {
    if (tshuf_layer(d)) return (int64_t)((d->cin + 15) / 16 * 16) * cout_pad(d->cout * (int)ipow(d->stride, d->ndim));
    int64_t per_axis = 0;
    for (int r = 0; r < d->stride; ++r) per_axis += tclass_axis(d, r).ke;
    return ipow(per_axis, d->ndim) * ((d->cin + 15) / 16 * 16) * cout_pad(d->cout);
}
bool im2col_layer(const s3r_conv_desc* d) {
    if (d->op != S3R_OP_CONV || !staged_layer(d) || d->cin > 8 || d->k > 16 || d->k < 2 || d->in_size > 4096) return false;
    const int no = out_size(d);
    if (no <= 0) return false;
    const double per_sample = ((double)d->cin * (double)ipow(d->k, d->ndim) + 15.0) * (d->ndim == 3 ? (double)no * no * no : (double)no * no);
    return per_sample * 4 <= 64.0 * (1 << 20);
}
StagedGeo staged_geo(const s3r_conv_desc* d) {
    StagedGeo s;
    s.bmax = 0;
    s.cin_pad = (d->cin + 15) / 16 * 16;
    if (im2col_layer(d)) {
        s.cin_pad = (d->cin * (int)ipow(d->k, d->ndim) + 15) / 16 * 16;
        s.step = 1; s.pe = 0;
        s.sp = out_size(d);
        const int64_t per_sample = (int64_t)s.cin_pad * ipow(s.sp, d->ndim);
        s.bmax = (int)(((int64_t)1 << 28) / per_sample);
        s.elems = (int64_t)(d->batch < s.bmax ? d->batch : s.bmax) * per_sample;
        return s;
    }
    if (tclass_layer(d)) {
        s.step = 1;
        s.pe = tclass_halo(d);
        s.sp = d->in_size + 2 * s.pe;
        s.elems = (int64_t)d->batch * s.cin_pad * ipow(s.sp, d->ndim);
        return s;
    }
    const bool tr = d->op == S3R_OP_DECONV;
    s.step = tr ? d->stride : 1;
    s.pe = tr ? dil_of(d) * (d->k - 1) - d->pad : d->pad;
    const int u = tr ? (d->in_size - 1) * d->stride + 1 + d->out_pad : d->in_size;
    s.sp = u + 2 * s.pe;
    s.elems = (int64_t)d->batch * s.cin_pad * ipow(s.sp, d->ndim);
    return s;
}

int geometry(const s3r_conv_desc* d, Geo* g) {
    if (!d) return fail(S3R_ERR_INVALID, "null descriptor");
    if (d->batch <= 0 || d->cin <= 0 || d->cout <= 0) return fail(S3R_ERR_INVALID, "batch/cin/cout must be positive");
    if (d->in_halo < 0 || d->out_halo < 0 || d->in_halo > 8 || d->out_halo > 8)
        return fail(S3R_ERR_INVALID, "halo must be in [0, 8]");
    if (d->dtype != S3R_F32 && d->dtype != S3R_BF16) return fail(S3R_ERR_INVALID, "unknown dtype %d", d->dtype);
    if ((d->in_layout != S3R_LAYOUT_PLAIN && d->in_layout != S3R_LAYOUT_WINO_H && d->in_layout != S3R_LAYOUT_WINO_DH &&
         d->in_layout != S3R_LAYOUT_WINO_HW && d->in_layout != S3R_LAYOUT_WINO_3D && d->in_layout != S3R_LAYOUT_DIFF) ||
        (d->out_layout != S3R_LAYOUT_PLAIN && d->out_layout != S3R_LAYOUT_WINO_HW && d->out_layout != S3R_LAYOUT_WINO_3D &&
         d->out_layout != S3R_LAYOUT_DIFF))
        return fail(S3R_ERR_INVALID, "unknown layout");
    if ((d->in_layout || d->out_layout) && d->op == S3R_OP_LINEAR)
        return fail(S3R_ERR_INVALID, "the transformed input layout exists on the convolution paths only");
    if (d->op == S3R_OP_LINEAR) {
        if (d->in_halo || d->out_halo) return fail(S3R_ERR_INVALID, "linear layers take no halo");
        if (d->act < S3R_ACT_NONE || d->act > S3R_ACT_TANH) return fail(S3R_ERR_INVALID, "unknown activation %d", d->act);
        g->nd = 0; g->in = g->out = g->in_p = g->out_p = 1; g->in_sp = 1; g->out_sp = 1;
        g->x_elems = (int64_t)d->batch * d->cin;
        g->y_elems = (int64_t)d->batch * d->cout;
        g->w_elems = (int64_t)d->cin * d->cout;
        g->x_store = g->x_elems; g->y_store = g->y_elems;
        g->flops = 2.0 * d->batch * (double)d->cin * d->cout;
        g->bytes = 4.0 * (g->x_elems + g->y_elems + g->w_elems);
        if (d->dtype != S3R_F32) return fail(S3R_ERR_INVALID, "linear layers exist on the fp32 path only");
        return S3R_OK;
    }
    if (d->op != S3R_OP_CONV && d->op != S3R_OP_DECONV) return fail(S3R_ERR_INVALID, "unknown op %d", d->op);
    if (d->ndim != 2 && d->ndim != 3) return fail(S3R_ERR_INVALID, "ndim must be 2 or 3");
    if (d->in_size <= 0 || d->k <= 0 || d->stride <= 0 || d->pad < 0) return fail(S3R_ERR_INVALID, "bad size/k/stride/pad");
    if (d->dilation < 0 || d->out_pad < 0) return fail(S3R_ERR_INVALID, "dilation / out_pad must not be negative");
    if (d->act < S3R_ACT_NONE || d->act > S3R_ACT_TANH) return fail(S3R_ERR_INVALID, "unknown activation %d", d->act);
    if (d->dtype == S3R_BF16 && (dil_of(d) != 1 || d->out_pad != 0 || d->act > S3R_ACT_SIGMOID || (d->op == S3R_OP_DECONV && !deconv_fast(d))))
        return fail(S3R_ERR_INVALID, "bf16 path: Conv with dilation 1 / ConvTranspose3d k4 s2 p1 and none / relu / sigmoid only (the "
                    "parameter-general layers are fp32)");
    if (d->op == S3R_OP_CONV && d->out_pad != 0) return fail(S3R_ERR_INVALID, "out_pad belongs to transposed convolutions");
    if (d->op == S3R_OP_DECONV && !deconv_fast(d)) {
        if (dil_of(d) * (d->k - 1) - d->pad < 0)
            return fail(S3R_ERR_INVALID, "ConvTranspose with pad %d > dilation * (k - 1) = %d crops more than the kernel reaches: not supported",
                        d->pad, dil_of(d) * (d->k - 1));
        if (d->out_pad >= (d->stride > dil_of(d) ? d->stride : dil_of(d)))
            return fail(S3R_ERR_INVALID, "out_pad %d must be smaller than max(stride, dilation)", d->out_pad);
    }
    if (staged_layer(d) && !im2col_layer(d)) {
        const bool tr = d->op == S3R_OP_DECONV && !tclass_layer(d);
        if (d->stride > 64 || d->k > 1024) return fail(S3R_ERR_INVALID, "stride / kernel size out of range");
        const double pe = tclass_layer(d) ? (double)tclass_halo(d) : tr ? (double)dil_of(d) * (d->k - 1) - d->pad : d->pad;
        const double sp = (tr ? ((double)d->in_size - 1) * d->stride + 1 + d->out_pad : d->in_size) + 2 * pe;
        const double est = (double)d->batch * ((d->cin + 15) / 16 * 16) * (d->ndim == 3 ? sp * sp * sp : sp * sp);
        if (est >= (double)kMaxElems || est * 4 >= (double)kMaxBytes)
            return fail(S3R_ERR_INVALID, "staged input too large for one call (>= 2^31 elements / 4 GiB): split the batch");
    }
    g->nd = d->ndim;
    g->in = d->in_size;
    g->out = out_size(d);
    if (g->out <= 0) return fail(S3R_ERR_INVALID, "empty output");
    g->in_p = g->in + 2 * d->in_halo;
    g->out_p = g->out + 2 * d->out_halo;
    g->in_sp = ipow(g->in, g->nd);
    g->out_sp = ipow(g->out, g->nd);
    g->x_elems = (int64_t)d->batch * d->cin * ipow(g->in_p, g->nd);
    g->y_elems = (int64_t)d->batch * d->cout * ipow(g->out_p, g->nd);
    if (d->in_layout == S3R_LAYOUT_WINO_H) {
        if (d->dtype != S3R_F32 || d->op != S3R_OP_CONV || d->stride != 1 || d->k != 3 || d->pad != 1 || (g->in & 1) || d->in_halo != 1 ||
            d->cin % 16 != 0 || d->cout <= 1)
            return fail(S3R_ERR_INVALID, "a Winograd-transformed input serves an fp32 Conv k=3 s=1 p=1 over an even edge, in_halo = 1");
        if (g->in % wino_r(d) != 0) return fail(S3R_ERR_INVALID, "a Winograd-transformed input needs an edge that is a multiple of %d", wino_r(d));
        g->x_elems = (wino_r(d) + 2) * (int64_t)d->batch * d->cin * (g->nd == 3 ? g->in_p : 1) * (g->in / wino_r(d)) * g->in_p;
    }
    if (d->in_layout == S3R_LAYOUT_WINO_DH) {
        if (d->dtype != S3R_F32 || d->op != S3R_OP_CONV || d->ndim != 3 || d->stride != 1 || d->k != 3 || d->pad != 1 || (g->in & 3) ||
            d->in_halo != 1 || d->cin % 32 != 0 || d->cout <= 1)
            return fail(S3R_ERR_INVALID, "a two-axis Winograd-transformed input serves an fp32 Conv3d k=3 s=1 p=1 over an edge %% 4 == 0, in_halo = 1");
        g->x_elems = 36 * (int64_t)d->batch * d->cin * (g->in / 4) * (g->in / 4) * g->in_p;
    }
    if (d->in_layout == S3R_LAYOUT_WINO_HW) {
        if (d->dtype != S3R_F32 || d->op != S3R_OP_CONV || d->ndim != 2 || d->stride != 1 || d->k != 3 || d->pad != 1 || (g->in & 3) ||
            d->in_halo != 1 || d->cin % 32 != 0 || d->cout <= 1)
            return fail(S3R_ERR_INVALID, "a two-axis Winograd-transformed input (2D) serves an fp32 Conv2d k=3 s=1 p=1 over an edge %% 4 == 0, in_halo = 1");
        g->x_elems = 36 * (int64_t)d->cin * s3r::wino2_npad((int64_t)d->batch * (g->in / 4) * (g->in / 4));
    }
    if (d->out_layout == S3R_LAYOUT_WINO_HW) {
        if (d->dtype != S3R_F32 || d->op != S3R_OP_CONV || d->ndim != 2 || (g->out & 3) || d->cout % 32 != 0 || d->act == S3R_ACT_SIGMOID)
            return fail(S3R_ERR_INVALID, "the two-axis Winograd output layout is written by an fp32 Conv2d with an output edge %% 4 == 0 and cout %% 32 == 0");
        g->y_elems = 36 * (int64_t)d->cout * s3r::wino2_npad((int64_t)d->batch * (g->out / 4) * (g->out / 4));
    }
    if (d->in_layout == S3R_LAYOUT_WINO_3D) {
        const int ax = wino2_ax(d);
        if ((ax != 0 && ax != 1) || d->in_halo != d->pad)
            return fail(S3R_ERR_INVALID, "the general two-axis Winograd input layout serves an fp32 Conv3d k=3 s=1 p=1 / k=4 s=1 p=0 with cin %% %d == 0, "
                        "in_halo = pad", s3r::wino_bk());
        g->x_elems = wino2_geo(d).v_sample * d->batch;
    }
    if (d->in_layout == S3R_LAYOUT_DIFF) {
        if (!dwino_layer(d) || d->in_halo != 1)
            return fail(S3R_ERR_INVALID, "the difference-tensor input layout serves the Winograd form of an fp32 ConvTranspose3d k=4 s=2 p=1 over an "
                        "edge %% 4 == 0, in_halo = 1");
        g->x_elems *= 4;
    }
    if (d->out_layout == S3R_LAYOUT_WINO_3D || d->out_layout == S3R_LAYOUT_DIFF) {
        const bool diff = d->out_layout == S3R_LAYOUT_DIFF;
        if (d->dtype != S3R_F32 || d->ndim != 3 || d->cout % s3r::wino_bk() != 0 || d->act > S3R_ACT_RELU ||
            (diff ? d->out_halo != 1 || (g->out & 3) : d->out_halo > 1 || g->out < (d->out_halo ? 4 : 5)))
            return fail(S3R_ERR_INVALID, "a consumer's operand is written by an fp32 3D layer with cout %% %d == 0, no activation or ReLU, and the halo the "
                        "consumer reads (two-axis planes: out_halo 1 for k3 p1, 0 for k4 p0; difference tensors: out_halo 1, output edge %% 4 == 0)",
                        s3r::wino_bk());
        if (diff) g->y_elems *= 4;
        else {
            const int sg = d->out_halo ? (g->out + 3) / 4 : (g->out - 2) / 2;
            g->y_elems = (int64_t)(d->out_halo ? 36 : 25) * d->batch * d->cout * sg * sg * g->out_p;
        }
    }
    g->w_elems = (int64_t)d->cin * d->cout * ipow(d->k, g->nd);
    if (d->op == S3R_OP_DECONV)
        g->flops = 2.0 * d->batch * (double)d->cin * g->in_sp * d->cout * ipow(d->k, g->nd);
    else
        g->flops = 2.0 * d->batch * (double)d->cout * g->out_sp * d->cin * ipow(d->k, g->nd);
    const bool bf = d->dtype == S3R_BF16;
    const bool stem = d->ndim == 2 && d->cin == 3;
    const bool head = d->cout == 1 && d->k == 1;
    const int xs = (bf && !stem) ? 2 : 4, ys = (bf && !head) ? 2 : 4, wsz = bf && !stem && !head ? 2 : 4;
    g->x_store = (g->x_elems * xs + 3) / 4;
    g->y_store = (g->y_elems * ys + 3) / 4;
    g->bytes = (double)d->batch * (xs * d->cin * (double)g->in_sp + ys * d->cout * (double)g->out_sp) + wsz * (double)g->w_elems;
    if (g->x_elems >= kMaxElems || g->y_elems >= kMaxElems || g->x_elems * 4 >= kMaxBytes || g->y_elems * 4 >= kMaxBytes)
        return fail(S3R_ERR_INVALID, "tensor too large for one call (>= 2^31 elements / 4 GiB): split the batch");
// ... 29 lines not shown
                    need_halo(d, r), d->in_halo);
    if ((r == R_STEM || r == R_HEAD) && d->in_halo != 0) return fail(S3R_ERR_INVALID, "stem / head kernels take an unpadded input");
    if (r == R_HEAD && d->out_halo != 0) return fail(S3R_ERR_INVALID, "head kernel writes an unpadded output");
    return S3R_OK;
}

int cout_pad(int cout) { return (cout + 127) / 128 * 128; }

int wino_mode() {
    static const int mode = getenv("S3R_WINO") ? atoi(getenv("S3R_WINO")) : 1;
    return mode;
}
bool wino_layer(const s3r_conv_desc* d) {
    return d->dtype != S3R_BF16 && d->op == S3R_OP_CONV && (d->ndim == 2 || d->ndim == 3) && d->k == 3 && d->stride == 1 &&
           d->pad == 1 && d->cin % s3r::wino_bk() == 0 && d->cout > 1 && d->in_size >= 4;
}
bool dwino_layer(const s3r_conv_desc* d) {
    return d->dtype != S3R_BF16 && deconv_fast(d) && d->cin % s3r::wino_bk() == 0 && d->in_size >= 4 && (d->in_size & 3) == 0;
}
bool dwino3_layer(const s3r_conv_desc* d) {
    return d->dtype != S3R_BF16 && deconv_fast(d) && d->cin % 16 == 0 && d->cout > 1 && s3r::dwino3_edge_ok(d->in_size);
}
bool dwino3_desc_ok(const s3r_conv_desc* d) {
    return dwino3_layer(d) && d->act < S3R_ACT_SIGMOID && d->in_halo == 1 && d->ksplit <= 1 && d->in_layout == S3R_LAYOUT_PLAIN &&
           d->out_layout == S3R_LAYOUT_PLAIN;
}
Dwino3Need dwino3_need(const s3r_conv_desc* d, int form) {
    Dwino3Need n;
    n.diff = (3 * (int64_t)d->batch * d->cin * ipow(d->in_size + 2, 3) + 255) / 256 * 256;
    const int ntotal = d->batch * (int)ipow(d->in_size / 2, 3);
    n.split = s3r::dwino3_split(d->cout, ntotal, form);
    n.total = n.diff + ((n.split || form < 0) ? (s3r::dwino3_slab_elems(d->cout, ntotal) + 255) / 256 * 256 : 0);
    return n;
}
int64_t dwino3_w_offset(const s3r_conv_desc* d) {
    return 64 * (int64_t)d->cin * cout_pad(d->cout) + (dwino_layer(d) ? dwino_w_elems(d) : 0);
}
bool wino_desc_ok(const s3r_conv_desc* d) {
    if (!(wino_layer(d) || dwino_layer(d)) || d->act >= S3R_ACT_SIGMOID || d->in_halo != 1 || d->ksplit > 1 || dil_of(d) != 1) return false;
    if (d->out_layout != S3R_LAYOUT_PLAIN && !(d->out_layout == S3R_LAYOUT_DIFF && dwino_layer(d))) return false;
    return d->in_layout == S3R_LAYOUT_PLAIN || (d->in_layout == S3R_LAYOUT_WINO_H && wino_layer(d)) ||
           (d->in_layout == S3R_LAYOUT_DIFF && dwino_layer(d));
}
int wino2_ax(const s3r_conv_desc* d) {
    if (d->dtype == S3R_BF16 || d->op != S3R_OP_CONV || d->stride != 1 || d->cin % s3r::wino_bk() != 0 || d->cout <= 1) return -1;
    if (d->ndim == 2) return d->k == 3 && d->pad == 1 && d->in_size >= 4 && d->in_size <= 124 ? 2 : -1;
    if (d->ndim != 3) return -1;
    if (d->k == 3 && d->pad == 1 && d->in_size >= 4) return 0;
    if (d->k == 4 && d->pad == 0 && d->in_size >= 5) return 1;
    return -1;
}
bool wino2_desc_ok(const s3r_conv_desc* d) {
    return wino2_ax(d) >= 0 && d->act < S3R_ACT_SIGMOID && dil_of(d) == 1 && d->in_halo == d->pad && d->ksplit <= 1 &&
           (d->in_layout == S3R_LAYOUT_PLAIN || (d->in_layout == S3R_LAYOUT_WINO_DH && wino2_ax(d) == 0 && d->in_size % 4 == 0) ||
            (d->in_layout == S3R_LAYOUT_WINO_HW && wino2_ax(d) == 2 && d->in_size % 4 == 0) ||
            (d->in_layout == S3R_LAYOUT_WINO_3D && wino2_ax(d) <= 1)) &&
           (d->out_layout == S3R_LAYOUT_PLAIN || (d->out_layout == S3R_LAYOUT_WINO_HW && wino2_ax(d) == 2 && d->in_size % 4 == 0) ||
            ((d->out_layout == S3R_LAYOUT_WINO_3D || d->out_layout == S3R_LAYOUT_DIFF) && wino2_ax(d) <= 1));
}
static bool forced_direct(const s3r_conv_desc* d) {
    return d->algo == S3R_ALGO_DIRECT || (d->algo == S3R_ALGO_AUTO && (d->tile >= 0 || d->ksplit >= 1));
}
static bool two_axis_io(const s3r_conv_desc* d) {
    if (d->in_layout == S3R_LAYOUT_WINO_DH || d->in_layout == S3R_LAYOUT_WINO_HW || d->in_layout == S3R_LAYOUT_WINO_3D ||
        d->out_layout == S3R_LAYOUT_WINO_HW)
        return true;
    return d->op == S3R_OP_CONV && (d->out_layout == S3R_LAYOUT_WINO_3D || d->out_layout == S3R_LAYOUT_DIFF) && wino2_ax(d) >= 0 &&
           !forced_direct(d);
}
int wino2_max_edge() {
    static const int e = getenv("S3R_WINO2_MAX_EDGE") ? atoi(getenv("S3R_WINO2_MAX_EDGE")) : 28;
    return e;
}
bool leaky_fused(const s3r_conv_desc* d) {
    return d->dtype == S3R_F32 && d->op != S3R_OP_LINEAR && d->act == S3R_ACT_LEAKY_RELU && d->act_param >= 0.f && d->act_param <= 1.f;
}
bool needs_act_pass(const s3r_conv_desc* d) { return d->act > S3R_ACT_SIGMOID && !leaky_fused(d); }

int resolve_algo(const s3r_conv_desc* d, int* alg, int* form) {
    *alg = ALG_DIRECT;
    *form = -1;
    if (d->algo != S3R_ALGO_AUTO && d->algo != S3R_ALGO_DIRECT && d->algo != S3R_ALGO_WINOGRAD)
        return fail(S3R_ERR_INVALID, "unknown algo %d", d->algo);
    if (staged_layer(d) || d->act > S3R_ACT_SIGMOID || dil_of(d) != 1) {
        if (d->algo == S3R_ALGO_WINOGRAD) return fail(S3R_ERR_INVALID, "algo = WINOGRAD: a parameter-general layer (staged input, dilation, "
                                                      "LeakyReLU / ELU / Tanh) has no Winograd form");
        if (d->in_layout != S3R_LAYOUT_PLAIN || d->out_layout != S3R_LAYOUT_PLAIN)
            return fail(S3R_ERR_INVALID, "a parameter-general layer reads and writes plain layouts");
        return S3R_OK;
    }
    if (d->algo == S3R_ALGO_WINOGRAD && d->tile >= 6 && d->tile <= 8) {
        if (!dwino3_desc_ok(d))
            return fail(S3R_ERR_INVALID, "algo = WINOGRAD, tile = 6: the three-axis form serves an fp32 ConvTranspose3d k4 s2 p1 over an edge of "
                        "8, 16 or 32 with cin %% 16 == 0 (in_halo = 1, plain layouts, no split-K, no sigmoid)");
        *alg = ALG_WINO3;
        *form = d->tile == 6 ? -1 : d->tile == 7 ? 1 : 0;
        return S3R_OK;
    }
    if (d->algo == S3R_ALGO_WINOGRAD) {
        const bool one = wino_desc_ok(d), two = wino2_desc_ok(d);
        if ((d->tile >= 3 && !two) || (d->tile >= 0 && d->tile <= 2 && !one) || (!one && !two) || d->tile > 5 ||
            (d->tile == 5 && (wino2_ax(d) == 1 || (wino2_ax(d) == 0 && d->in_size > 60))))
            return fail(S3R_ERR_INVALID, "algo = WINOGRAD: this layer / descriptor has no such Winograd form (one-axis: fp32 Conv k3 s1 p1 "
                        "with cin %% %d == 0 and edge >= 4, or ConvTranspose3d k4 s2 p1 over an edge %% 4 == 0, in_halo = 1; two-axis "
                        "(tile = 3): Conv3d k3 s1 p1 / k4 s1 p0, in_halo = pad; plain layouts, no split-K, no sigmoid)", s3r::wino_bk());
        const bool two_io = two_axis_io(d);
        if (two_io && !(two && (d->tile < 0 || d->tile >= 3)))
            return fail(S3R_ERR_INVALID, "a two-axis transformed input / output runs the two-axis kernel only");
        if (d->tile >= 3 || !one || two_io ||
            (d->tile < 0 && two && d->in_layout == S3R_LAYOUT_PLAIN && d->in_size <= wino2_max_edge())) {
            *alg = ALG_WINO2;
            *form = d->tile >= 4 ? d->tile - 4 : -1;
        } else { *alg = ALG_WINO; *form = d->tile; }
        return S3R_OK;
    }
    if (two_axis_io(d)) {
        if (d->algo == S3R_ALGO_DIRECT || !wino2_desc_ok(d) || d->tile >= 0)
// ... 68 lines not shown
int64_t dwino_d_elems(const s3r_conv_desc* d) {
    return (dwino_materialise(d) ? 3 : 1) * (int64_t)d->batch * d->cin * ipow(d->in_size + 2, 3);
}

int wino_kind(const s3r_conv_desc* d) { return d->op == S3R_OP_DECONV ? 2 : 1; }
int wino_kcls(const s3r_conv_desc* d) {
    return d->cin * (d->op == S3R_OP_DECONV ? 2 : (d->ndim == 3 ? 9 : 3));
}
int64_t wino_positions(const s3r_conv_desc* d, int nb) {
    const int n = d->in_size;
    if (d->op == S3R_OP_DECONV) return (int64_t)nb * (n / 2) * (n / 2) * n;
    const int R = wino_r(d);
    return (int64_t)nb * (d->ndim == 3 ? n : 1) * ((n + R - 1) / R) * n;
}
WinoNeed wino_need(const s3r_conv_desc* d, int form, bool head) {
    WinoNeed w = {0, 0, 0};
    if (d->batch <= 0) return w;
    const int kind = wino_kind(d);
    if (d->op == S3R_OP_DECONV) {
        if (d->in_layout != S3R_LAYOUT_DIFF) w.v = dwino_d_elems(d);
        const int nt = (int)wino_positions(d, d->batch);
        w.slab = s3r::wino_slab_elems(kind, d->cout, nt, s3r::wino_plan(kind, d->cout, wino_kcls(d), nt, head, form < 0 ? 1 : form));
    } else {
        const int bmax = wino_bmax(d);
        if (bmax <= 0) return w;
        if (d->in_layout != S3R_LAYOUT_WINO_H) w.v = wino_v_elems(d) / d->batch * bmax;
        for (int b0 = 0; b0 < d->batch; b0 += bmax) {
            const int nb = d->batch - b0 < bmax ? d->batch - b0 : bmax;
            if (b0 > 0 && nb == bmax) continue;
            const int nt = (int)wino_positions(d, nb);
            const int64_t sl = s3r::wino_slab_elems(kind, d->cout, nt, s3r::wino_plan(kind, d->cout, wino_kcls(d), nt, false, form < 0 ? 1 : form));
            if (sl > w.slab) w.slab = sl;
        }
    }
    w.v = (w.v + 255) / 256 * 256;
    w.total = w.v + w.slab;
    return w;
}
double wino_exec_flops(const s3r_conv_desc* d, const Geo& g) {
    if (d->op == S3R_OP_DECONV) return g.flops * 0.5625;
    const int R = wino_r(d);
    const double taps = (d->ndim == 3 ? 3.0 : 1.0) * 3.0 * (R + 2);
    return 2.0 * (double)wino_positions(d, d->batch) * d->cout * d->cin * taps;
}

int wino2_form_of(const s3r_conv_desc* d, int ntotal, int forced) {
    if (forced < 0 && wino2_ax(d) == 0 && d->in_size > 60) forced = 0;
    return s3r::wino2_form(wino2_ax(d), d->cout, ntotal, forced);
}
WinoNeed wino2_need(const s3r_conv_desc* d, int form) {
    WinoNeed w = {0, 0, 0};
    const Wino2Geo g2 = wino2_geo(d);
    if (d->batch <= 0 || g2.bmax <= 0) return w;
    if (d->in_layout != S3R_LAYOUT_WINO_DH && d->in_layout != S3R_LAYOUT_WINO_HW && d->in_layout != S3R_LAYOUT_WINO_3D)
        w.v = ((g2.ax == 2 ? g2.ncls * d->cin * s3r::wino2_npad(g2.pos_sample * g2.bmax) : g2.v_sample * g2.bmax) + 255) / 256 * 256;
    for (int b0 = 0; b0 < d->batch; b0 += g2.bmax) {
        const int nb = d->batch - b0 < g2.bmax ? d->batch - b0 : g2.bmax;
        if (b0 > 0 && nb == g2.bmax) continue;
        const int nt = (int)(g2.pos_sample * nb);
        const int64_t sl = s3r::wino2_slab_elems(g2.ax, d->cout, nt, form < 0 ? 0 : wino2_form_of(d, nt, form));
        if (sl > w.slab) w.slab = sl;
    }
    w.total = w.v + w.slab;
    return w;
}
double wino2_exec_flops(const s3r_conv_desc* d) {
    const Wino2Geo g2 = wino2_geo(d);
    return 2.0 * (double)g2.pos_sample * d->batch * g2.ncls * d->cout * d->cin * g2.kw;
}
int cout_pad_h(int cout) { return (cout + 63) / 64 * 64; }

s3r::ConvParamsH make_params_h(const s3r_conv_desc* d, const Geo& g) {
    s3r::ConvParamsH p;
    memset(&p, 0, sizeof(p));
    const bool is3 = d->ndim == 3;
    p.B = d->batch; p.Cin = d->cin; p.Cout = d->cout; p.CoutPad = cout_pad_h(d->cout);
    p.act = d->act;
    p.x_ws = d->cin; p.x_hs = g.in_p * d->cin; p.x_ds = is3 ? g.in_p * g.in_p * d->cin : 0;
    p.x_bs = (int)ipow(g.in_p, g.nd) * d->cin;
    p.y_ws = d->cout; p.y_hs = g.out_p * d->cout; p.y_ds = is3 ? g.out_p * g.out_p * d->cout : 0;
    p.y_bs = (int)ipow(g.out_p, g.nd) * d->cout;
    p.y_org = d->out_halo * (p.y_ds + p.y_hs + p.y_ws);
    p.x_bytes = (unsigned)(g.x_elems * 2);
    if (d->op == S3R_OP_DECONV) {
        p.transposed = 1;
        p.Nd = g.in; p.Nh = g.in; p.Nw = g.in;
        p.kd = p.kh = p.kw = 2; p.T = 8;
        p.stride = 1;
        p.x_org = d->in_halo * (p.x_ds + p.x_hs + p.x_ws);
    } else {
        p.transposed = 0;
        p.Nd = is3 ? g.out : 1; p.Nh = g.out; p.Nw = g.out;
        p.kd = is3 ? d->k : 1; p.kh = d->k; p.kw = d->k; p.T = p.kd * p.kh * p.kw;
        p.stride = d->stride;
        p.x_org = (d->in_halo - d->pad) * (p.x_ds + p.x_hs + p.x_ws);
    }
    p.Ntotal = p.B * p.Nd * p.Nh * p.Nw;
    p.dS = s3r::FastDiv((unsigned)(p.Nd * p.Nh * p.Nw));
    p.dHW = s3r::FastDiv((unsigned)(p.Nh * p.Nw));
    p.dW = s3r::FastDiv((unsigned)p.Nw);
    p.dDH = s3r::FastDiv((unsigned)(p.Nd * p.Nh));
    p.dH = s3r::FastDiv((unsigned)p.Nh);
    p.ksplit = 1;
    return p;
}


int resolve_launch_h(const s3r_conv_desc* d, s3r::ConvParamsH* p, LaunchH* L) {
    const int chunks = d->cin / 32;
    if (d->ksplit < 0 || (d->ksplit > 0 && chunks % d->ksplit != 0))
        return fail(S3R_ERR_INVALID, "ksplit=%d must divide cin/32=%d", d->ksplit, chunks);
    L->ksplit = d->ksplit > 0 ? d->ksplit : s3r::conv_bf16_pick_ksplit(*p);
    p->ksplit = L->ksplit;
    if (d->tile >= 0 && d->tile != 1 && d->tile != 2 && d->tile != 3 && d->tile != 19 && d->tile != 4 && d->tile != 5 && d->tile != 6 && d->tile != 9 &&
        d->tile != 10 && d->tile != 17 && d->tile != 18 && d->tile != 20 && d->tile != 21 && d->tile != 22 && d->tile != 23 &&
        d->tile != 40)
        return fail(S3R_ERR_INVALID, "bf16 path: tile must be -1 (auto), 1, 2, 4 (x128 positions, per-tap gather), 3 (128 x 128 couts), 5, 6 "
                    "(x128 positions = 1, 2, plane-reuse gather) or 9, 10 (row-reuse gather); per-tap / plane + 16 = "
                    "32-channel K tiles; 40 (row-persistent e2)");
    L->tm = d->tile >= 0 ? d->tile : s3r::conv_bf16_pick_tm(*p);
    return S3R_OK;
// ... 112 lines not shown
        taps_before = (is3 ? kd_before * sum_ke * sum_ke : 0) + (int64_t)ad.ke * kh_before * sum_ke + (int64_t)ad.ke * ah.ke * kw_before;
    }
    *w_off = taps_before * sg.cin_pad * cout_pad(d->cout);
    if (ad.nq <= 0 || ah.nq <= 0 || aw.nq <= 0) return false;
    s3r::ConvParams p = make_params(d, g);
    p.Cin = sg.cin_pad;
    p.transposed = 0;
    p.x_hs = sg.sp; p.x_ds = is3 ? sg.sp * sg.sp : 0; p.x_cs = (int)ipow(sg.sp, g.nd);
    p.x_bytes = (unsigned)(sg.elems * 4);
    p.Nd = is3 ? ad.nq : 1; p.Nh = ah.nq; p.Nw = aw.nq;
    p.kd = is3 ? ad.ke : 1; p.kh = ah.ke; p.kw = aw.ke; p.T = p.kd * p.kh * p.kw;
    p.stride = 1; p.dil = 1;
    p.x_org = (is3 ? (h + ad.qmin - (ad.ke - 1)) * p.x_ds : 0) + (h + ah.qmin - (ah.ke - 1)) * p.x_hs + (h + aw.qmin - (aw.ke - 1));
    p.y_step = s;
    p.y_org += (is3 ? (s * ad.qmin + rd - d->pad) * p.y_ds : 0) + (s * ah.qmin + rh - d->pad) * p.y_hs + (s * aw.qmin + rw - d->pad);
    p.Ntotal = p.B * p.Nd * p.Nh * p.Nw;
    p.dS = s3r::FastDiv((unsigned)(p.Nd * p.Nh * p.Nw));
    p.dHW = s3r::FastDiv((unsigned)(p.Nh * p.Nw));
    p.dW = s3r::FastDiv((unsigned)p.Nw);
    p.ksplit = 1;
    *macs = (double)p.Ntotal * p.T * (double)sg.cin_pad * d->cout;
    *q = p;
    return true;
}


int resolve_launch(const s3r_conv_desc* d, s3r::ConvParams* p, Launch* L) {
    const int chunks = d->cin / 16;
    if (d->ksplit < 0 || (d->ksplit > 0 && chunks % d->ksplit != 0))
        return fail(S3R_ERR_INVALID, "ksplit=%d must divide cin/16=%d", d->ksplit, chunks);
    L->ksplit = d->ksplit > 0 ? d->ksplit : s3r::conv_pick_ksplit(*p, 0);
    p->ksplit = L->ksplit;
    const int code = d->tile >= 0 ? d->tile : 15;
    L->cfg = code & 15;
    L->vec = code >> 4;
    if (L->cfg != 15 && L->cfg >= s3r::conv_num_tiles()) return fail(S3R_ERR_INVALID, "unknown tile configuration %d", L->cfg);
    if (L->cfg == 15) L->cfg = s3r::conv_pick_tile(*p);
    const int vmax = s3r::conv_pick_vec(*p);
    const int vec = (L->vec == 1 || L->vec == 4) && L->vec <= vmax ? L->vec : vmax;
    int bm, bn;
    s3r::conv_tile_dims(L->cfg, &bm, &bn);
    if (bn > 256 * vec)
        return fail(S3R_ERR_INVALID, "tile configuration %d (%d positions) needs the 16-byte gather: rows of a multiple of 4 positions, "
                    "stride 1", L->cfg, bn);
    return S3R_OK;
}


int64_t align_up(int64_t v, int64_t a) { return (v + a - 1) / a * a; }

static int handoff_mask() {
    static const int m = getenv("S3R_WINO_HANDOFF") ? atoi(getenv("S3R_WINO_HANDOFF")) : 1;
    return m == 1 ? ~0 : m;
}

static int handoff3d(const s3r_conv_desc& a, const s3r_conv_desc& b, bool* take) {
    *take = false;
    if (a.dtype != S3R_F32 || b.dtype != S3R_F32 || a.ndim != 3 || b.ndim != 3 || a.cout != b.cin || out_size(&a) != b.in_size ||
        a.batch != b.batch || a.out_halo != b.in_halo || a.act > S3R_ACT_RELU || a.cout % s3r::wino_bk() != 0 || staged_layer(&a) ||
        staged_layer(&b))
        return S3R_LAYOUT_PLAIN;
    const int op = b.in_size + 2 * b.in_halo;
    if (op * op * op > 8192) return S3R_LAYOUT_PLAIN;
    int alg_a, form_a, alg_b, form_b;
    if (resolve_algo(&a, &alg_a, &form_a) != S3R_OK || resolve_algo(&b, &alg_b, &form_b) != S3R_OK) return S3R_LAYOUT_PLAIN;
    int lay = S3R_LAYOUT_PLAIN, bit = 0;
    bool forms = true;
    if (alg_b == ALG_WINO2 && wino2_ax(&b) <= 1 && b.in_halo == b.pad && b.in_size >= (b.pad ? 4 : 5) && wino2_geo(&b).bmax >= b.batch)
        lay = S3R_LAYOUT_WINO_3D;
    else if (alg_b == ALG_WINO && b.op == S3R_OP_DECONV && b.in_halo == 1 && dwino_materialise(&b))
        lay = S3R_LAYOUT_DIFF;
    else return S3R_LAYOUT_PLAIN;
    if (alg_a == ALG_WINO2 && wino2_ax(&a) <= 1) {
        bit = lay == S3R_LAYOUT_DIFF ? 16 : 8;
        const Wino2Geo g2 = wino2_geo(&a);
        if (g2.bmax < a.batch) return S3R_LAYOUT_PLAIN;
        forms = wino2_form_of(&a, (int)(g2.pos_sample * a.batch), form_a) == 0;
    } else if (alg_a == ALG_WINO && a.op == S3R_OP_DECONV && lay == S3R_LAYOUT_DIFF) {
        bit = 32;
        forms = s3r::wino_plan(2, a.cout, wino_kcls(&a), (int)wino_positions(&a, a.batch), false, form_a).mode == s3r::WINO_CP;
    } else if (alg_a == ALG_DIRECT && a.op == S3R_OP_CONV && lay == S3R_LAYOUT_WINO_3D && a.out_layout == S3R_LAYOUT_PLAIN) {
        bit = 4;
        Geo ga;
        Launch L;
        if (geometry(&a, &ga) != S3R_OK) return S3R_LAYOUT_PLAIN;
        s3r::ConvParams pa = make_params(&a, ga);
        if (resolve_launch(&a, &pa, &L) != S3R_OK || L.ksplit <= 1) return S3R_LAYOUT_PLAIN;
    } else return S3R_LAYOUT_PLAIN;
    if (!(handoff_mask() & bit)) return S3R_LAYOUT_PLAIN;
    s3r_conv_desc a2 = a, b2 = b;
    a2.out_layout = lay; b2.in_layout = lay;
    int alg2, form2;
    Geo g2;
    if (geometry(&a2, &g2) != S3R_OK || geometry(&b2, &g2) != S3R_OK) return S3R_LAYOUT_PLAIN;
    if (resolve_algo(&a2, &alg2, &form2) != S3R_OK || alg2 != alg_a || form2 != form_a) return S3R_LAYOUT_PLAIN;
    if (resolve_algo(&b2, &alg2, &form2) != S3R_OK || alg2 != alg_b || form2 != form_b) return S3R_LAYOUT_PLAIN;
    *take = forms;
    return lay;
}

int plan_chain(const s3r_layer* layers, int n, Plan* pl) {
    if (!layers || n <= 0) return fail(S3R_ERR_INVALID, "empty chain");
    pl->d.resize(n); pl->r.resize(n); pl->g.resize(n); pl->off.assign(n, -1); pl->fuse_head.assign(n, 0); pl->region.assign(n, 0);
    for (int i = 0; i < n; ++i) {
        pl->d[i] = layers[i].desc;
        if (i > 0) pl->d[i].in_layout = S3R_LAYOUT_PLAIN;
// ... 182 lines not shown

}

extern "C" {

int64_t s3r_chain_workspace_elems(const s3r_layer* layers, int n_layers) {
    Plan pl;
    int rc = plan_chain(layers, n_layers, &pl);
    if (rc) return rc;
    return pl.total;
}

static int wino_input_layout(const s3r_conv_desc* d, int64_t* elems) {
    *elems = 0;
    if (!d) return S3R_LAYOUT_PLAIN;
    s3r_conv_desc t = *d;
    t.in_layout = S3R_LAYOUT_PLAIN;
    int alg, form;
    if (resolve_algo(&t, &alg, &form) != S3R_OK || t.op != S3R_OP_CONV) return S3R_LAYOUT_PLAIN;
    if (alg == ALG_WINO && t.in_size % wino_r(&t) == 0 && wino_bmax(&t) >= t.batch) {
        *elems = wino_v_elems(&t);
        return S3R_LAYOUT_WINO_H;
    }
    if (alg == ALG_WINO2 && wino2_ax(&t) == 0 && t.in_size % 4 == 0) {
        const Wino2Geo g2 = wino2_geo(&t);
        if (g2.bmax >= t.batch) {
            *elems = g2.v_sample * t.batch;
            return S3R_LAYOUT_WINO_DH;
        }
    }
    if (alg == ALG_WINO2 && wino2_ax(&t) == 2 && t.in_size % 4 == 0) {
        const Wino2Geo g2 = wino2_geo(&t);
        if (g2.bmax >= t.batch) {
            *elems = g2.ncls * t.cin * s3r::wino2_npad(g2.pos_sample * t.batch);
            return S3R_LAYOUT_WINO_HW;
        }
    }
    return S3R_LAYOUT_PLAIN;
}

int64_t s3r_conv_wino_input_elems(const s3r_conv_desc* d) {
    if (!d) return fail(S3R_ERR_INVALID, "null descriptor");
    int64_t elems;
    (void)wino_input_layout(d, &elems);
    return elems;
}

int s3r_conv_wino_input_layout(const s3r_conv_desc* d) {
    if (!d) return fail(S3R_ERR_INVALID, "null descriptor");
    int64_t elems;
    return wino_input_layout(d, &elems);
}

}
```

stereo-3d-reconstruction_amd/modules.py:

```python
from __future__ import annotations

import collections
import ctypes as C
import dataclasses
import os
import weakref
from typing import Dict, List, Optional, Sequence

import torch
import torch.nn as nn

from . import _lib
from . import arch_spec as spec

MAX_CHUNK = 256

_DEBUG = {"tile": {}, "ksplit": {}, "algo": {}}


class debug_overrides:

    def __init__(self, tile=None, ksplit=None, algo=None):
        self._new = {"tile": dict(tile or {}), "ksplit": dict(ksplit or {}), "algo": dict(algo or {})}
        for kind, d in self._new.items():
# ... 228 lines not shown
            arr[i].packed_w = pw.data_ptr()
            arr[i].scale = scale.data_ptr() if scale is not None else None
            arr[i].shift = shift.data_ptr() if shift is not None else None
        return arr, n_layers

    def _has_winograd_form(self, l: spec.Layer) -> bool:
        if self.precision != "fp32" or l.op not in ("conv2d", "conv3d", "deconv3d"):
            return False
        n_in = self._sizes()[self.names.index(l.name)][0]
        desc = _lib.make_desc(l, 1, n_in, in_halo=1 if l.op == "deconv3d" else l.p, dtype=self._dtype, algo=_lib.ALGO_WINOGRAD)
        return _lib.load().s3r_conv_scratch_elems(C.byref(desc)) >= 0

    def _tile_ksplit_of(self, l: spec.Layer):
        return (int(_DEBUG["tile"].get(l.name, self.tile_override.get(l.name, -1))),
                int(_DEBUG["ksplit"].get(l.name, self.ksplit_override.get(l.name, 0))))

    def _algo_of(self, l: spec.Layer) -> int:
        if l.name in _DEBUG["algo"]:
            return int(_DEBUG["algo"][l.name])
        if l.name in self.algo_override:
            return int(self.algo_override[l.name])
        if self.winograd is None:
            return _lib.ALGO_AUTO
        if self.winograd and self._has_winograd_form(l):
            return _lib.ALGO_WINOGRAD
        return _lib.ALGO_DIRECT

    def wino_input_layout(self, batch: int) -> int:
        if self.precision != "fp32" or batch <= 0:
            return _lib.LAYOUT_PLAIN
        l, (n_in, _) = self._layers[0], self._sizes()[0]
        tile, ksplit = self._tile_ksplit_of(l)
        desc = _lib.make_desc(l, batch, n_in, tile=tile, in_halo=1, ksplit=ksplit, dtype=self._dtype, algo=self._algo_of(l))
        return _lib.check(_lib.load().s3r_conv_wino_input_layout(C.byref(desc)), "wino_input_layout")

    def takes_wino_input(self, batch: int) -> bool:
        return self.wino_input_layout(batch) != _lib.LAYOUT_PLAIN

    def _out_shape(self, batch: int, n_layers: int):
        l = self._layers[n_layers - 1]
        m = self._sizes()[n_layers - 1][1]
        nd = spec.ndim(l)
        return (batch, l.cout) + (m,) * nd

    def _out_is_bf16(self, n_layers: int) -> bool:
        l = self._layers[n_layers - 1]
        return self.precision == "bf16" and not (l.cout == 1 and l.k == 1)

    @torch.no_grad()
    def _run(self, x: torch.Tensor, upto: Optional[str] = None, in_halo: int = 0,
             x2: Optional[torch.Tensor] = None, in_layout: int = 0) -> torch.Tensor:
        lib = _lib.load()
        device, batch = x.device, x.shape[0] + (x2.shape[0] if x2 is not None else 0)
        if in_layout in (_lib.LAYOUT_WINO_H, _lib.LAYOUT_WINO_DH):
            batch = x.shape[1]
        if batch == 0:
            n0 = len(self._layers) if upto is None else self.names.index(upto) + 1
            shape = self._out_shape(0, n0)
            if self._out_is_bf16(n0):
                return _to_logical(torch.empty((0,) + shape[2:] + (shape[1],), dtype=torch.bfloat16, device=device))
            return torch.empty(shape, dtype=torch.float32, device=device)
        arr, n = self._layer_array(batch, device, upto, in_halo, in_layout)
        shape = self._out_shape(batch, n)
        if self._out_is_bf16(n):
            y = torch.empty((shape[0],) + shape[2:] + (shape[1],), dtype=torch.bfloat16, device=device)
        else:
            y = torch.empty(shape, dtype=torch.float32, device=device)
        need = _lib.check(lib.s3r_chain_workspace_elems(arr, n), "workspace query")
        cfg = tuple((arr[i].desc.tile, arr[i].desc.ksplit, arr[i].desc.algo) for i in range(n)) + (in_layout,)
        ws, fresh = self._ws.get(device, need, (batch, n, in_halo, need, cfg))
        u8 = x.dtype == torch.uint8
        if (u8 or x2 is not None) and self._entry != "s3r_encoder_forward":
            raise RuntimeError("8-bit renders / a (left, right) tensor pair are inputs of the encoder only")
        if x2 is not None and x2.dtype != x.dtype:
            raise RuntimeError("left and right renders must share one dtype")
        if x2 is not None or u8:
            enc = lib.s3r_encoder_forward_u8 if u8 else lib.s3r_encoder_forward
            _lib.check(enc(arr, n, x.data_ptr(), x2.data_ptr() if x2 is not None else None, y.data_ptr(), ws.data_ptr(),
                           ws.numel(), fresh, _stream_ptr(device)), type(self).__name__)
        elif upto is None and self._entry == "s3r_encoder_forward":
            _lib.check(lib.s3r_encoder_forward(arr, n, x.data_ptr(), None, y.data_ptr(), ws.data_ptr(), ws.numel(), fresh,
                                               _stream_ptr(device)), type(self).__name__)
        else:
            entry = getattr(lib, self._entry if upto is None else "s3r_chain_forward")
            _lib.check(entry(arr, n, x.data_ptr(), y.data_ptr(), ws.data_ptr(), ws.numel(), fresh, _stream_ptr(device)),
                       type(self).__name__)
        return _to_logical(y) if self._out_is_bf16(n) else y


    _TUNE_TILES = (1, 2, 3, 7, 0)
    _TUNE_TILES_BF16 = (1, 3, 9, 17, 22, 23)
    _TUNE_KSPLITS = (1, 2, 4, 8)

    def _differentiable_layers(self, x: torch.Tensor, first: int, stop: int, batch_stats: bool = False) -> torch.Tensor:
        n_in = self._sizes()[first][0]
        x = _check_input(x, "x", (self._layers[first].cin,) + (n_in,) * 3)
        for l in self._layers[first:stop]:
            blk: _Block = getattr(self, l.name)
            if batch_stats and blk.bn is not None:
                z = differentiable_conv(x, blk.conv.weight, None, blk.conv.bias, dataclasses.replace(l, act="none"))
                x = differentiable_batchnorm(z, blk.bn, l.act)
                continue
            scale, _ = blk.folded()
            if scale is None:
                shift = blk.conv.bias
            else:
                shift = blk.bn.bias + (blk.conv.bias - blk.bn.running_mean.detach()) * scale
# ... 90 lines not shown
        if B:
            _lib.check(_lib.load().s3r_cost_volume_forward_bf16(fl.data_ptr(), fr.data_ptr(), vol.data_ptr(), B, Cc,
                                                                self.max_disp, H, W, halo, _stream_ptr(fl.device)),
                       "cost_volume (bf16)")
        return vol

    @torch.no_grad()
    def forward_padded(self, feat_left: torch.Tensor, feat_right: torch.Tensor, halo: int = 1) -> torch.Tensor:
        if self.precision == "bf16":
            return self._bf16(feat_left, feat_right, halo, resident=True)
        fl = _check_input(feat_left, "feat_left", feat_left.shape[1:])
        fr = _check_input(feat_right, "feat_right", feat_left.shape[1:])
        B, Cc, H, W = fl.shape
        shape = (B, 2 * Cc, self.max_disp + 2 * halo, H + 2 * halo, W + 2 * halo)
        if self._padded is None or tuple(self._padded.shape) != shape or self._padded.device != fl.device:
            if getattr(self, "_pinned", False):
                raise RuntimeError("the padded cost volume of this module is captured in a HIP graph for another shape")
            self._padded = torch.zeros(shape, dtype=torch.float32, device=fl.device)
        if B == 0:
            return self._padded
        _lib.check(_lib.load().s3r_cost_volume_forward(fl.data_ptr(), fr.data_ptr(), self._padded.data_ptr(), B, Cc,
                                                       self.max_disp, H, W, halo, _stream_ptr(fl.device)),
                   "cost_volume")
        return self._padded

    @torch.no_grad()
    def forward_wino(self, feat_left: torch.Tensor, feat_right: torch.Tensor) -> torch.Tensor:
        fl = _check_input(feat_left, "feat_left", feat_left.shape[1:])
        fr = _check_input(feat_right, "feat_right", feat_left.shape[1:])
        B, Cc, H, W = fl.shape
        shape = (6, B, 2 * Cc, self.max_disp + 2, H // 4, W + 2)
        if self._planes is None or tuple(self._planes.shape) != shape or self._planes.device != fl.device:
            if getattr(self, "_pinned", False):
                raise RuntimeError("the padded cost volume of this module is captured in a HIP graph for another shape")
            self._planes = torch.zeros(shape, dtype=torch.float32, device=fl.device)
        _lib.check(_lib.load().s3r_cost_volume_forward_wino(fl.data_ptr(), fr.data_ptr(), self._planes.data_ptr(), B, Cc,
                                                            self.max_disp, H, W, _stream_ptr(fl.device)), "cost_volume (wino)")
        return self._planes

    @torch.no_grad()
    def forward_wino2(self, feat_left: torch.Tensor, feat_right: torch.Tensor) -> torch.Tensor:
        fl = _check_input(feat_left, "feat_left", feat_left.shape[1:])
        fr = _check_input(feat_right, "feat_right", feat_left.shape[1:])
        B, Cc, H, W = fl.shape
        shape = (36, B, 2 * Cc, self.max_disp // 4, H // 4, W + 2)
        if self._planes is None or tuple(self._planes.shape) != shape or self._planes.device != fl.device:
            if getattr(self, "_pinned", False):
                raise RuntimeError("the padded cost volume of this module is captured in a HIP graph for another shape")
            self._planes = torch.zeros(shape, dtype=torch.float32, device=fl.device)
        _lib.check(_lib.load().s3r_cost_volume_forward_wino2(fl.data_ptr(), fr.data_ptr(), self._planes.data_ptr(), B, Cc,
                                                             self.max_disp, H, W, _stream_ptr(fl.device)), "cost_volume (wino2)")
        return self._planes

    def forward_for(self, consumer, feat_left: torch.Tensor, feat_right: torch.Tensor):
        layout = consumer.wino_input_layout(feat_left.shape[0])
        if layout == _lib.LAYOUT_WINO_H:
            return self.forward_wino(feat_left, feat_right), layout
        if layout == _lib.LAYOUT_WINO_DH:
            return self.forward_wino2(feat_left, feat_right), layout
        return self.forward_padded(feat_left, feat_right), _lib.LAYOUT_PLAIN

    @torch.no_grad()
    def forward(self, feat_left: torch.Tensor, feat_right: torch.Tensor) -> torch.Tensor:
        if self.precision == "bf16":
            return _to_logical(self._bf16(feat_left, feat_right, 0, resident=False))
        if feat_left.shape != feat_right.shape or feat_left.dim() != 4:
            raise RuntimeError(f"feature maps must both be (B,C,H,W), got {tuple(feat_left.shape)} and "
                               f"{tuple(feat_right.shape)}")
        fl = _check_input(feat_left, "feat_left", feat_left.shape[1:])
        fr = _check_input(feat_right, "feat_right", feat_left.shape[1:])
        B, Cc, H, W = fl.shape
        vol = torch.empty((B, 2 * Cc, self.max_disp, H, W), dtype=torch.float32, device=fl.device)
        if B == 0:
            return vol
        _lib.check(_lib.load().s3r_cost_volume_forward(fl.data_ptr(), fr.data_ptr(), vol.data_ptr(), B, Cc,
                                                       self.max_disp, H, W, 0, _stream_ptr(fl.device)), "cost_volume")
        return vol

    def differentiable(self, feat_left: torch.Tensor, feat_right: torch.Tensor) -> torch.Tensor:
        if self.precision != "fp32":
            raise RuntimeError(f"CostVolume.differentiable is implemented for fp32 models only (this one is {self.precision}): the "
                               "cost-volume backward kernel reads fp32 tensors")
        return differentiable_cost_volume(feat_left, feat_right, self.max_disp)


def _check_wino_planes(v: torch.Tensor, layout: int = _lib.LAYOUT_WINO_H) -> torch.Tensor:
    if layout == _lib.LAYOUT_WINO_DH:
        ncls, want = 36, (2 * spec.FEAT_C, spec.MAX_DISP // 4, spec.FEAT_HW // 4, spec.FEAT_HW + 2)
    else:
        ncls, want = 6, (2 * spec.FEAT_C, spec.MAX_DISP + 2, spec.FEAT_HW // 4, spec.FEAT_HW + 2)
    if not isinstance(v, torch.Tensor) or not v.is_cuda or v.dtype != torch.float32 or v.dim() != 6 or v.shape[0] != ncls or \
            tuple(v.shape[2:]) != want or not v.is_contiguous():
        raise RuntimeError(f"transformed volume must be a contiguous float32 HIP tensor ({ncls}, B, {', '.join(map(str, want))})")
    return v


class Decoder(_HipChain):
    _entry = "s3r_decoder_forward"

    def __init__(self, precision: str = "fp32", winograd=None):
        super().__init__(spec.DECODER, spec.MAX_DISP, tag_base=200, precision=precision, winograd=winograd)

    def forward(self, volume: torch.Tensor, upto: Optional[str] = None) -> torch.Tensor:
        tail = (2 * spec.FEAT_C, spec.MAX_DISP, spec.FEAT_HW, spec.FEAT_HW)
        if self.precision == "bf16":
            x = _check_input_cl(volume, "volume", tail)
        else:
            x = _check_input(volume, "volume", tail)
        y = self._run(x, upto)
        return y.squeeze(1) if upto is None or upto == self.names[-1] else y

    def forward_padded(self, volume_padded: torch.Tensor, halo: int = 1, in_layout: int = 0, upto: Optional[str] = None) -> torch.Tensor:
        last = upto is None or upto == self.names[-1]
        if in_layout in (_lib.LAYOUT_WINO_H, _lib.LAYOUT_WINO_DH):
            y = self._run(_check_wino_planes(volume_padded, in_layout), upto, in_halo=1, in_layout=in_layout)
            return y.squeeze(1) if last else y
        n = (spec.MAX_DISP + 2 * halo, spec.FEAT_HW + 2 * halo, spec.FEAT_HW + 2 * halo)
        if self.precision == "bf16":
            x = _check_input(volume_padded, "volume_padded", n + (2 * spec.FEAT_C,), torch.bfloat16)
        else:
            x = _check_input(volume_padded, "volume_padded", (2 * spec.FEAT_C,) + n)
        y = self._run(x, upto, in_halo=halo)
        return y.squeeze(1) if last else y

    FEATURES = "d3"

    def _fp32_only(self, what: str):
        if self.precision != "fp32":
            raise RuntimeError(f"{what} is implemented for fp32 models only (this one is {self.precision}): the head backward and the "
                               "BCE kernels read fp32 tensors")

    def features(self, volume: torch.Tensor) -> torch.Tensor:
        self._fp32_only("Decoder.features")
        return self.forward(volume, upto=self.FEATURES)

    def differentiable_head(self, features: torch.Tensor) -> torch.Tensor:
        self._fp32_only("Decoder.differentiable_head")
        l = self._layers[-1]
        x = _check_input(features, "features", (l.cin,) + (spec.VOX,) * 3)
        blk: _Block = getattr(self, l.name)
        return differentiable_head(x, blk.conv.weight, blk.conv.bias, l.act)

    def differentiable_features(self, x: torch.Tensor, start: str = "d3", batch_stats: bool = False) -> torch.Tensor:
        self._fp32_only("Decoder.differentiable_features")
        if start not in self.names[:-1]:
            raise RuntimeError(f"start must be one of {self.names[:-1]}, got {start!r}")
        return self._differentiable_layers(x, self.names.index(start), len(self._layers) - 1, batch_stats)

    def differentiable_tail(self, x: torch.Tensor, start: str = "d3", batch_stats: bool = False) -> torch.Tensor:
        self._fp32_only("Decoder.differentiable_tail")
        return self.differentiable_head(self.differentiable_features(x, start, batch_stats))


class VolumeEncoder(_HipChain):
    _entry = "s3r_decoder_forward"

    def __init__(self, precision: str = "fp32", winograd=None):
        super().__init__(spec.DECODER_DOWN, spec.MAX_DISP, tag_base=200, precision=precision, winograd=winograd)

    def forward(self, volume: torch.Tensor) -> torch.Tensor:
        tail = (2 * spec.FEAT_C, spec.MAX_DISP, spec.FEAT_HW, spec.FEAT_HW)
        if self.precision == "bf16":
            return self._run(_check_input_cl(volume, "volume", tail))
        return self._run(_check_input(volume, "volume", tail))

    def forward_padded(self, volume_padded: torch.Tensor, halo: int = 1, in_layout: int = 0) -> torch.Tensor:
        if in_layout in (_lib.LAYOUT_WINO_H, _lib.LAYOUT_WINO_DH):
            return self._run(_check_wino_planes(volume_padded, in_layout), None, in_halo=1, in_layout=in_layout)
        n = (spec.MAX_DISP + 2 * halo, spec.FEAT_HW + 2 * halo, spec.FEAT_HW + 2 * halo)
        if self.precision == "bf16":
            x = _check_input(volume_padded, "volume_padded", n + (2 * spec.FEAT_C,), torch.bfloat16)
        else:
            x = _check_input(volume_padded, "volume_padded", (2 * spec.FEAT_C,) + n)
        return self._run(x, None, in_halo=halo)

    def differentiable_features(self, x: torch.Tensor, start: str = "v1", batch_stats: bool = False) -> torch.Tensor:
        if self.precision != "fp32":
            raise RuntimeError(f"VolumeEncoder.differentiable_features is implemented for fp32 models only (this one is "
                               f"{self.precision}): the conv backward kernels read fp32 tensors")
        if start not in self.names:
            raise RuntimeError(f"start must be one of {self.names}, got {start!r}")
        return self._differentiable_layers(x, self.names.index(start), len(self._layers), batch_stats)


class PointHead(_HipChain):

    def __init__(self):
        super().__init__(spec.POINT_HEAD, 1, tag_base=300)

    def forward(self, latent: torch.Tensor) -> torch.Tensor:
        x = _check_input(latent, "latent", (spec.LATENT_C, 4, 4, 4))
        return self._run(x.view(x.shape[0], spec.LATENT_C * 64)).view(x.shape[0], spec.N_POINTS, 3)

    def differentiable(self, latent: torch.Tensor) -> torch.Tensor:
        x = _check_input(latent, "latent", (spec.LATENT_C, 4, 4, 4))
        h = x.view(x.shape[0], spec.LATENT_C * 64)
        for l in self._layers:
            blk: _Block = getattr(self, l.name)
            h = differentiable_linear(h, blk.conv.weight, blk.conv.bias, l.act)
        return h.view(x.shape[0], spec.N_POINTS, 3)


DISPARITY_TEMPERATURE = 1.0

READOUTS = ("wta", "soft")


class _DisparityMixin:

    disparity_temperature = DISPARITY_TEMPERATURE

    @torch.no_grad()
    def disparity(self, left: torch.Tensor, right: torch.Tensor, in_pixels: bool = True, readout: str = "wta",
                  temperature: Optional[float] = None, full_resolution: bool = False, confidence: bool = False):
        if readout not in READOUTS:
            raise ValueError(f"readout must be one of {READOUTS}, got {readout!r}")
        if readout == "wta" and (full_resolution or confidence or temperature is not None):
            raise ValueError("full_resolution / confidence / temperature need readout='soft' (the WTA read-out is integer, "
                             "at feature resolution)")
        if readout == "soft":
# ... 27 lines not shown
        parts = []
        for s in range(0, max(left.shape[0], 1), MAX_CHUNK):
            l, r = left[s:s + MAX_CHUNK], right[s:s + MAX_CHUNK]
            b = l.shape[0]
            feats = self.encoder.forward_pair(l, r)
            parts.append(disparity_soft(feats[:b], feats[b:], self.cost_volume.max_disp, tau, size, scale, confidence))
        return tuple(p[0] if len(parts) == 1 else torch.cat(p, 0) for p in zip(*parts))

    @torch.no_grad()
    def stereo_features(self, left: torch.Tensor, right: torch.Tensor):
        if self.precision != "fp32":
            raise RuntimeError(f"stereo_features is implemented for fp32 models only (this one is {self.precision}): the cost-volume "
                               "backward kernel reads fp32 tensors")
        left = _check_render(left, "left")
        right = _check_render(right, "right")
        if left.shape[0] != right.shape[0]:
            raise RuntimeError("left and right batch sizes differ")
        fls, frs = [], []
        for s in range(0, max(left.shape[0], 1), MAX_CHUNK):
            l, r = left[s:s + MAX_CHUNK], right[s:s + MAX_CHUNK]
            b = l.shape[0]
            feats = self.encoder.forward_pair(l, r)
            fls.append(feats[:b]), frs.append(feats[b:])
        if len(fls) == 1:
            return fls[0].clone(), frs[0].clone()
        return torch.cat(fls, 0), torch.cat(frs, 0)


class Stereo2Voxel(_DisparityMixin, nn.Module):

    def __init__(self, precision: str = "fp32", winograd=None):
        super().__init__()
        self.precision = precision
        self.winograd = winograd
        self.encoder = Encoder(precision, winograd)
        self.cost_volume = CostVolume(precision=precision)
        self.decoder = Decoder(precision, winograd)
        self.eval()

    def train(self, mode: bool = True):
        if mode:
            raise RuntimeError("forward/inference path only")
        return super().train(False)

    def _decoded(self, left: torch.Tensor, right: torch.Tensor, upto: Optional[str] = None):
        left = _check_render(left, "left")
        right = _check_render(right, "right")
        if left.shape[0] != right.shape[0]:
            raise RuntimeError("left and right batch sizes differ")
        for s in range(0, max(left.shape[0], 1), MAX_CHUNK):
            l, r = left[s:s + MAX_CHUNK], right[s:s + MAX_CHUNK]
            b = l.shape[0]
            feats = self.encoder.forward_pair(l, r)
            vol, layout = self.cost_volume.forward_for(self.decoder, feats[:b], feats[b:])
            yield self.decoder.forward_padded(vol, in_layout=layout, upto=upto)

    @torch.no_grad()
    def forward(self, left: torch.Tensor, right: torch.Tensor) -> torch.Tensor:
        outs = list(self._decoded(left, right))
        return outs[0] if len(outs) == 1 else torch.cat(outs, 0)

    @torch.no_grad()
    def trunk_features(self, left: torch.Tensor, right: torch.Tensor, upto: str = "d2") -> torch.Tensor:
        self.decoder._fp32_only("Stereo2Voxel.trunk_features")
        if upto not in self.decoder.names[:-1]:
            raise RuntimeError(f"upto must be one of {self.decoder.names[:-1]}, got {upto!r}")
        outs = list(self._decoded(left, right, upto=upto))
        return outs[0] if len(outs) == 1 else torch.cat(outs, 0)

    @torch.no_grad()
    def head_features(self, left: torch.Tensor, right: torch.Tensor) -> torch.Tensor:
        self.decoder._fp32_only("Stereo2Voxel.head_features")
        return self.trunk_features(left, right, upto=Decoder.FEATURES)

    @torch.no_grad()
    def autotune(self, left: torch.Tensor, right: torch.Tensor, rounds: int = 3, log=None):
        b = left.shape[0]
        images = torch.cat([left, right], 0)
        chosen = dict(self.encoder.autotune(images, rounds=rounds, log=log))
        feats = self.encoder(images)
        vol = self.cost_volume.forward_padded(feats[:b], feats[b:])
        chosen.update(self.decoder.autotune(vol, in_halo=1, rounds=rounds, log=log))
        return chosen


class Stereo2Point(_DisparityMixin, nn.Module):

    def __init__(self, precision: str = "fp32", winograd=None):
        super().__init__()
        self.precision = precision
        self.winograd = winograd
        self.encoder = Encoder(precision, winograd)
        self.cost_volume = CostVolume(precision=precision)
        self.decoder = VolumeEncoder(precision, winograd)
        self.point_head = PointHead()
        self.eval()

    def train(self, mode: bool = True):
        if mode:
            raise RuntimeError("forward/inference path only")
        return super().train(False)

    def _latents(self, left: torch.Tensor, right: torch.Tensor):
        left = _check_render(left, "left")
        right = _check_render(right, "right")
        if left.shape[0] != right.shape[0]:
            raise RuntimeError("left and right batch sizes differ")
        for s in range(0, max(left.shape[0], 1), MAX_CHUNK):
            l, r = left[s:s + MAX_CHUNK], right[s:s + MAX_CHUNK]
            b = l.shape[0]
            feats = self.encoder.forward_pair(l, r)
            vol, layout = self.cost_volume.forward_for(self.decoder, feats[:b], feats[b:])
            latent = self.decoder.forward_padded(vol, in_layout=layout)
            if latent.dtype != torch.float32:
                latent = channels_last_to_f32(latent)
            yield latent

    @torch.no_grad()
    def forward(self, left: torch.Tensor, right: torch.Tensor) -> torch.Tensor:
        outs = [self.point_head(latent) for latent in self._latents(left, right)]
        return outs[0] if len(outs) == 1 else torch.cat(outs, 0)

    @torch.no_grad()
    def latent(self, left: torch.Tensor, right: torch.Tensor) -> torch.Tensor:
        outs = list(self._latents(left, right))
        return outs[0] if len(outs) == 1 else torch.cat(outs, 0)


_LINEAR_ACTS = ("none", "relu", "sigmoid")


def _check_linear(x, weight, act, who):
    if act not in _LINEAR_ACTS:
        raise RuntimeError(f"{who}: act must be one of {_LINEAR_ACTS}, got {act!r}")
    if x.dim() != 2 or weight.dim() != 2 or x.shape[1] != weight.shape[1]:
        raise RuntimeError(f"{who} expects x (B,Cin) and weight (Cout,Cin), got {tuple(x.shape)} and {tuple(weight.shape)}")
    x = _check_input(x, "x", (weight.shape[1],))
    w = weight.detach()
    if w.device != x.device or w.dtype != torch.float32 or not w.is_contiguous():
        raise RuntimeError(f"{who}: weight must be a contiguous fp32 tensor on {x.device}")
    if w.numel() == 0:
        raise RuntimeError(f"{who} needs a non-empty weight")
    return x, w


@torch.no_grad()
def linear(x: torch.Tensor, weight: torch.Tensor, bias: Optional[torch.Tensor], act: str = "none") -> torch.Tensor:
    x, w = _check_linear(x, weight, act, "linear")
    B, cin, cout = x.shape[0], w.shape[1], w.shape[0]
    b = None
    if bias is not None:
        b = bias.detach()
        if b.shape != (cout,) or b.device != x.device or b.dtype != torch.float32 or not b.is_contiguous():
            raise RuntimeError(f"linear: bias must be a contiguous fp32 ({cout},) tensor on {x.device}")
    y = torch.empty((B, cout), dtype=torch.float32, device=x.device)
    if B:
        lib = _lib.load()
        need = _lib.check(lib.s3r_linear_scratch_elems(B, cin, cout), "linear scratch query")
        scratch = torch.empty(max(need, 1), dtype=torch.float32, device=x.device)
        _lib.check(lib.s3r_linear_forward(x.data_ptr(), w.data_ptr(), None if b is None else b.data_ptr(), y.data_ptr(), B, cin, cout,
                                          _lib.ACT[act], scratch.data_ptr(), scratch.numel(), _stream_ptr(x.device)), "linear")
    return y


@torch.no_grad()
# ... 722 lines not shown
```

Baseline: 8833.

## Skip structurally-zero cost-volume halves in the first Winograd 3D conv

Adds a cost-volume-aware input layout in which positions are regrouped cell-major by column-quad zones per depth group. The first two-axis Winograd conv can then skip whole Cin halves (left or right features) that are provably zero because disparity exceeds the column. Zeros are structural to the cost volume, not to the data, so no required work is dropped. This cuts the GEMM K-loop for many tiles of the first decoder conv, in exchange for more complex index decoding in the B-load and output scatter paths and a new layout that must stay consistent.

```diff
diff --git a/include/s3r.h b/include/s3r.h
--- a/include/s3r.h
+++ b/include/s3r.h
@@ -32,7 +32,7 @@
                        S3R_ACT_LEAKY_RELU = 3, S3R_ACT_ELU = 4, S3R_ACT_TANH = 5  } s3r_act;
 
 typedef enum s3r_layout { S3R_LAYOUT_PLAIN = 0, S3R_LAYOUT_WINO_H = 2, S3R_LAYOUT_WINO_DH = 3, S3R_LAYOUT_WINO_HW = 4,
-                          S3R_LAYOUT_WINO_3D = 5, S3R_LAYOUT_DIFF = 6 } s3r_layout;
+                          S3R_LAYOUT_WINO_3D = 5, S3R_LAYOUT_DIFF = 6, S3R_LAYOUT_WINO_DH_CV = 7 } s3r_layout;
 
 typedef enum s3r_algo { S3R_ALGO_AUTO = 0, S3R_ALGO_DIRECT = 1, S3R_ALGO_WINOGRAD = 2 } s3r_algo;
 
@@ -98,6 +98,8 @@
 int s3r_conv_wino_input_layout(const s3r_conv_desc* d);
 int s3r_cost_volume_forward_wino2(const float* feat_left, const float* feat_right, float* planes, int batch, int channels,
                                   int max_disp, int height, int width, void* stream);
+int s3r_cv_zero_skip(int in_size, int depth_group, int column_quad, int depth_class);
+int s3r_cv_column_group(int in_size, int depth_group, int column_quad);
 
 int s3r_cost_volume_forward_bf16(const void* feat_left, const void* feat_right, void* volume, int batch, int channels,
                                  int max_disp, int height, int width, int out_halo, void* stream);
diff --git a/stereo-3d-reconstruction_amd/_lib.py b/stereo-3d-reconstruction_amd/_lib.py
--- a/stereo-3d-reconstruction_amd/_lib.py
+++ b/stereo-3d-reconstruction_amd/_lib.py
@@ -72,6 +72,8 @@
     "s3r_conv_wino_input_layout": (C.c_int, [C.POINTER(ConvDesc)]),
     "s3r_cost_volume_forward_wino2": (C.c_int, [C.c_void_p, C.c_void_p, C.c_void_p, C.c_int, C.c_int, C.c_int, C.c_int,
                                                 C.c_int, C.c_void_p]),
+    "s3r_cv_zero_skip": (C.c_int, [C.c_int, C.c_int, C.c_int, C.c_int]),
+    "s3r_cv_column_group": (C.c_int, [C.c_int, C.c_int, C.c_int]),
     "s3r_cost_volume_backward": (C.c_int, [C.c_void_p, C.c_void_p, C.c_void_p, C.c_int, C.c_int, C.c_int, C.c_int, C.c_int,
                                            C.c_void_p]),
     "s3r_linear_scratch_elems": (C.c_int64, [C.c_int, C.c_int, C.c_int]),
@@ -144,7 +146,7 @@
     return rc
 
 
-LAYOUT_PLAIN, LAYOUT_WINO_H, LAYOUT_WINO_DH, LAYOUT_WINO_HW, LAYOUT_WINO_3D, LAYOUT_DIFF = 0, 2, 3, 4, 5, 6
+LAYOUT_PLAIN, LAYOUT_WINO_H, LAYOUT_WINO_DH, LAYOUT_WINO_HW, LAYOUT_WINO_3D, LAYOUT_DIFF, LAYOUT_WINO_DH_CV = 0, 2, 3, 4, 5, 6, 7
 
 
 def make_desc(layer, batch, in_size, tag=0, tile=-1, in_halo=0, out_halo=0, ksplit=0, dtype=0, in_layout=0, out_layout=0,
diff --git a/stereo-3d-reconstruction_amd/csrc/s3r_api.hip b/stereo-3d-reconstruction_amd/csrc/s3r_api.hip
--- a/stereo-3d-reconstruction_amd/csrc/s3r_api.hip
+++ b/stereo-3d-reconstruction_amd/csrc/s3r_api.hip
@@ -17,8 +17,9 @@
               int64_t scratch_elems, int form, hipStream_t s, int* launches) {
     const Wino2Geo g2 = wino2_geo(d);
     const WinoNeed need = wino2_need(d, form);
-    const bool pre = d->in_layout == S3R_LAYOUT_WINO_DH || d->in_layout == S3R_LAYOUT_WINO_HW ||
+    const bool pre = layout_dh(d->in_layout) || d->in_layout == S3R_LAYOUT_WINO_HW ||
                      d->in_layout == S3R_LAYOUT_WINO_3D;
+    p.cv = cv_zero_used(d) ? 1 : 0;
     const bool to_v = d->out_layout == S3R_LAYOUT_WINO_HW;
     p.out_mode = d->out_layout == S3R_LAYOUT_WINO_3D ? (d->out_halo ? 1 : 2) : d->out_layout == S3R_LAYOUT_DIFF ? 3 : 0;
     if (p.out_mode && (g2.ax > 1 || wino2_form_of(d, (int)(g2.pos_sample * d->batch), form) != 0))
diff --git a/stereo-3d-reconstruction_amd/csrc/s3r_conv_wino.hip b/stereo-3d-reconstruction_amd/csrc/s3r_conv_wino.hip
--- a/stereo-3d-reconstruction_amd/csrc/s3r_conv_wino.hip
+++ b/stereo-3d-reconstruction_amd/csrc/s3r_conv_wino.hip
@@ -1,5 +1,6 @@
 #include "s3r_kernels.h"
 #include <cstdlib>
+#include <vector>
 
 namespace s3r {
 
@@ -236,7 +237,7 @@
     return t;
 }
 
-template <int VEC, int KIND, int WN, bool CP, bool HEAD, bool XM = false, bool SEMI = false>
+template <int VEC, int KIND, int WN, bool CP, bool HEAD, bool XM = false, bool SEMI = false, bool CV = false>
 __device__ __forceinline__ void wino_body(const ConvParams& p, const int bid_in, const int nwg_in, const int n_begin,
                                           const int n_end, float* __restrict__ wsmem) {
     constexpr bool DECONV = KIND == 2;
@@ -247,6 +248,7 @@
     static_assert(!SEMI || (KIND == 1 && !CP && !HEAD), "the semi-fused form: serial F(4,3) row classes of one depth class");
     static_assert(WN == 4 || WN == 2, "4 waves as 1 x 4 or 2 x 2");
     static_assert(!HEAD || (DECONV && !CP && WN == 2), "the fused head: serial transposed form");
+    static_assert(!CV || (KIND == 1 && VEC == 4 && (CP || SEMI)), "cell-major positions: the two-axis 3D forms, column quads");
     float* As = wsmem;
     constexpr int BSTG = (DECONV ? 2 : 1) * WBK * BN;
     float* Bs = wsmem + WNB * WBK * WBM;
@@ -296,7 +298,31 @@
     const int S = p.Nd * p.Nh * p.Nw;
     const int T = DECONV ? 2 : p.T;
     const int chunks = p.Cin / WBK;
-    const int nkt = T * chunks;
+    int cc_lo = 0, cc_hi = chunks;
+    if constexpr (CV) {
+        const int n_last = (n0 + BN < n_end ? n0 + BN : n_end) - 1;
+        const int a = cls0 / NCLS, edge = p.Nw;
+        int b_, sd0, sh_, pw_, q0, gw, sd1, q1, gw1;
+        cv_decode(p, n0, b_, sd0, sh_, pw_, q0, gw);
+        cv_decode(p, n_last, b_, sd1, sh_, pw_, q1, gw1);
+        int live = 0;
+        for (int sd = sd0; sd <= sd1 && live != 3; ++sd) {
+            int lo, hi;
+            cv_zones(sd, edge >> 2, lo, hi);
+            const int zb[4] = {0, lo, hi, edge >> 2};
+#pragma unroll
+            for (int z = 0; z < 3; ++z) {
+                if (zb[z] == zb[z + 1] || (sd == sd0 && zb[z] < q0) || (sd == sd1 && zb[z] > q1)) continue;
+                live |= cv_live_halves(sd, zb[z], a, edge, zb[z + 1] - 1);
+            }
+        }
+        live = __builtin_amdgcn_readfirstlane(live);
+        cc_lo = (live & 1) ? 0 : chunks >> 1;
+        cc_hi = (live & 2) ? chunks : chunks >> 1;
+        if (!live) cc_hi = cc_lo;
+    }
+    const int nkt = T * (cc_hi - cc_lo);
+    const int nkt_skip = T * chunks - nkt;
     const int total = NACC * nkt;
 
     int bvoff;
@@ -306,12 +332,18 @@
         else        { col = (lane % LPR_B) * VEC;           lrow = lane / LPR_B; }
         int n = n0 + col;
         if (n >= n_end) n = n_end - VEC;
-        const int b = p.dS.div(n);
-        int rem = n - b * S;
-        const int pd = p.dHW.div(rem);
-        rem -= pd * p.Nh * p.Nw;
-        const int q = p.dW.div(rem);
-        const int pw = rem - q * p.Nw;
+        int b, pd, q, pw;
+        if constexpr (CV) {
+            int q0_, gw_;
+            cv_decode(p, n, b, pd, q, pw, q0_, gw_);
+        } else {
+            b = p.dS.div(n);
+            int rem = n - b * S;
+            pd = p.dHW.div(rem);
+            rem -= pd * p.Nh * p.Nw;
+            q = p.dW.div(rem);
+            pw = rem - q * p.Nw;
+        }
         if constexpr (DECONV)
             bvoff = (b * p.Cin * p.x_cs + (2 * pd + rd) * p.x_ds + (2 * q + rh) * p.x_hs + pw + rw + lrow * p.x_cs) * 4;
         else
@@ -333,8 +365,8 @@
     constexpr int B_LDS_STEP = B_WIDE ? B_ROW_STEP * BN : 4 * PB;
     const int cs4 = p.x_cs * 4;
 
-    int c_cls = cls0, c_cc = 0, c_td = 0, c_tw = 0, c_tap = 0;
-    int c_kt = (DECONV ? pc * NCLS + cls0 : cls0) * nkt;
+    int c_cls = cls0, c_cc = cc_lo, c_td = 0, c_tw = 0, c_tap = 0;
+    int c_kt = (DECONV ? pc * NCLS + cls0 : cls0) * (T * chunks) + cc_lo * T;
     int c_a = cls0 / 3, c_b = cls0 - 3 * (cls0 / 3);
 #ifdef S3R_ABLATE
     bool abl_loop = false;
@@ -397,7 +429,10 @@
             if (++c_tw == p.kw) { c_tw = 0; ++c_td; }
             if (++c_tap == T) {
                 c_tap = 0; c_td = 0; c_tw = 0;
-                if (++c_cc == chunks) { c_cc = 0; ++c_cls; }
+                if (++c_cc == cc_hi) {
+                    c_cc = cc_lo; ++c_cls;
+                    if constexpr (CV) c_kt += nkt_skip;
+                }
             }
         }
     };
@@ -627,10 +662,10 @@
 }
 #undef S3R_TL_FINISH
 
-template <int VEC, int KIND, int WN, bool CP, bool HEAD, bool XM = false, bool SEMI = false>
+template <int VEC, int KIND, int WN, bool CP, bool HEAD, bool XM = false, bool SEMI = false, bool CV = false>
 __global__ __launch_bounds__(256, (CP || KIND == 1 ? 4 : 3)) void wino_kernel(const ConvParams p) {
     extern __shared__ __attribute__((aligned(16))) float wsmem[];
-    wino_body<VEC, KIND, WN, CP, HEAD, XM, SEMI>(p, blockIdx.x, gridDim.x, p.n_begin, p.n_end, wsmem);
+    wino_body<VEC, KIND, WN, CP, HEAD, XM, SEMI, CV>(p, blockIdx.x, gridDim.x, p.n_begin, p.n_end, wsmem);
 }
 
 template <int VEC, int KIND, bool HEAD = false, bool XM = false>
@@ -1023,11 +1058,24 @@
         for (int t = tid; t < nsub * G; t += 256) {
             const int sub = p.dHW.div(t);
             const int g = t - sub * G;
-            const int sh = p.dW.div(g);
-            const int pw = g - sh * p.Nw;
+            int sh = p.dW.div(g);
+            int pw = g - sh * p.Nw;
             const int r = r0 + sub;
-            const int sd = r - dNd.div(r) * p.Nd;
-            const int n = r0 * G + t;
+            const int bb = dNd.div(r);
+            const int sd = r - bb * p.Nd;
+            int n = r0 * G + t;
+            if (p.cv) {
+                const int nq = p.Nw >> 2, unit = p.Nh * 4;
+                int lo, hi;
+                cv_zones(sd, nq, lo, hi);
+                const int q0 = g < unit * lo ? 0 : g < unit * hi ? lo : hi;
+                const int gw = g < unit * lo ? lo : g < unit * hi ? hi - lo : nq - hi;
+                const int rem = g - unit * q0;
+                sh = (int)((unsigned)rem / (unsigned)(4 * gw));
+                const int wl = rem - sh * 4 * gw;
+                pw = 4 * q0 + wl;
+                n = sd * (p.B * p.Nh * p.Nw) + p.B * unit * q0 + (bb * p.Nh + sh) * 4 * gw + wl;
+            }
             const float* __restrict__ src = p.part + ((size_t)mrow * (npad >> 6) + (n >> 6)) * (N * M * 64) + (n & 63);
             float* __restrict__ o = fsm + sub * MS + (halo + M * sh) * Wp + halo + pw;
 #pragma unroll
@@ -1077,12 +1125,18 @@
     for (long long i = (long long)blockIdx.x * 256 + threadIdx.x; i < total; i += (long long)gridDim.x * 256) {
         const int mrow = (int)(i / nn);
         const int n = (int)(i - (long long)mrow * nn);
-        const int b = p.dS.div(n);
-        int rem = n - b * S;
-        const int sd = p.dHW.div(rem);
-        rem -= sd * p.Nh * p.Nw;
-        const int sh = p.dW.div(rem);
-        const int pw = rem - sh * p.Nw;
+        int b, sd, sh, pw;
+        if (p.cv) {
+            int q0_, gw_;
+            cv_decode(p, n, b, sd, sh, pw, q0_, gw_);
+        } else {
+            b = p.dS.div(n);
+            int rem = n - b * S;
+            sd = p.dHW.div(rem);
+            rem -= sd * p.Nh * p.Nw;
+            sh = p.dW.div(rem);
+            pw = rem - sh * p.Nw;
+        }
         const float* __restrict__ src = p.part + ((size_t)mrow * (npad >> 6) + (n >> 6)) * (N * N * 64) + (n & 63);
         float t[N][M];
 #pragma unroll
@@ -1544,6 +1598,45 @@
     return semi_wgs >= (ax == 2 ? 2 : 8) * (long)cu_count() ? 1 : 0;
 }
 int64_t wino2_npad(int64_t ntotal) { return (ntotal + WCN - 1) / WCN * WCN; }
+static void cv_group_of(int sd, int nq, int q, int* q0, int* gw) {
+    int lo, hi;
+    cv_zones(sd, nq, lo, hi);
+    if (q < lo) { *q0 = 0; *gw = lo; } else if (q < hi) { *q0 = lo; *gw = hi - lo; } else { *q0 = hi; *gw = nq - hi; }
+}
+int wino2_cv_group(int edge, int sd, int q) {
+    int q0, gw;
+    cv_group_of(sd, edge / 4, q, &q0, &gw);
+    return q0;
+}
+double wino2_cv_live_share(int batch, int edge) {
+    if (batch <= 0 || edge < 4 || edge % 4 != 0) return 1.0;
+    const int nq = edge / 4;
+    std::vector<int> grp;
+    for (int sd = 0; sd < nq; ++sd)
+        for (int q = 0; q < nq;) {
+            int q0, gw;
+            cv_group_of(sd, nq, q, &q0, &gw);
+            grp.insert(grp.end(), (size_t)batch * nq * gw, sd * nq + q0);
+            q = q0 + gw;
+        }
+    long long live = 0, all = 0;
+    for (size_t t0 = 0; t0 < grp.size(); t0 += WCN / 4) {
+        const size_t t1 = t0 + WCN / 4 < grp.size() ? t0 + WCN / 4 : grp.size();
+        for (int a = 0; a < 6; ++a) {
+            int m = 0, prev = -1;
+            for (size_t t = t0; t < t1; ++t) {
+                if (grp[t] == prev) continue;
+                prev = grp[t];
+                int q0, gw;
+                cv_group_of(prev / nq, nq, prev % nq, &q0, &gw);
+                m |= cv_live_halves(prev / nq, q0, a, edge, q0 + gw - 1);
+            }
+            live += (m & 1) + ((m >> 1) & 1);
+            all += 2;
+        }
+    }
+    return (double)live / (double)all;
+}
 int64_t wino2_slab_elems(int ax, int cout, int ntotal, int form) {
     const int64_t npad = (int64_t)((ntotal + WCN - 1) / WCN) * WCN;
     return (form ? 6 * 4 : wino2_classes(ax)) * (int64_t)cout * npad;
@@ -1551,7 +1644,7 @@
 
 hipError_t launch_conv_wino2(ConvParams p, int ax, int form, bool to_v, hipStream_t stream, int* launches) {
     if (p.Cin % WBK != 0 || p.stride != 1 || p.transposed || p.ksplit != 1 || p.head_w || p.act == ACT_SIGMOID || !p.part ||
-        ax < 0 || ax > 2 || p.ncls != wino2_classes(ax))
+        ax < 0 || ax > 2 || p.ncls != wino2_classes(ax) || (p.cv && ax != 0))
         return hipErrorInvalidValue;
     p.kh = 1;
     S3R_WABL(p);
@@ -1595,6 +1688,12 @@
         return hipGetLastError();
     }
     if (p.y_ds != p.y_hs * p.y_hs || p.y_cs != (p.Dout + 2 * halo) * p.y_ds) return hipErrorInvalidValue;
+    if (p.cv) {
+        if (ax != 0 || p.out_mode || p.Nw % 4 != 0 || p.Nd * 4 != p.Nw || p.Nh != p.Nd || p.Cin % (2 * WBK) != 0) return hipErrorInvalidValue;
+        p.cv = 1;
+        p.dCvSd = FastDiv((unsigned)(p.B * p.Nh * p.Nw));
+        p.dCvSH = FastDiv((unsigned)p.Nh);
+    }
     if (form == 1) {
         const int M = wino2_outputs(ax), G = p.Nh * p.Nw;
         if (ax != 0 || (size_t)M * p.y_ds * 4 > 64 * 1024) return hipErrorInvalidValue;
@@ -1606,7 +1705,8 @@
         const long long items = (long long)p.Cout * ((p.B * p.Nd + SUB - 1) / SUB);
         const dim3 fgrid((unsigned)(items < 32768 ? items : 32768));
         const dim3 grid(p.m_tiles * n_tiles * 6);
-        if (p.Nw % 4 == 0) hipLaunchKernelGGL((wino_kernel<4, 1, 2, false, false, false, true>), grid, dim3(256), lds, stream, p);
+        if (p.cv) hipLaunchKernelGGL((wino_kernel<4, 1, 2, false, false, false, true, true>), grid, dim3(256), lds, stream, p);
+        else if (p.Nw % 4 == 0) hipLaunchKernelGGL((wino_kernel<4, 1, 2, false, false, false, true>), grid, dim3(256), lds, stream, p);
         else hipLaunchKernelGGL((wino_kernel<1, 1, 2, false, false, false, true>), grid, dim3(256), lds, stream, p);
         hipError_t e = hipGetLastError();
         if (e != hipSuccess) return e;
@@ -1616,7 +1716,8 @@
         return hipGetLastError();
     }
     const dim3 grid(p.m_tiles * n_tiles * p.ncls);
-    if (p.Nw % 4 == 0) hipLaunchKernelGGL((wino_kernel<4, 1, 2, true, false>), grid, dim3(256), lds, stream, p);
+    if (p.cv) hipLaunchKernelGGL((wino_kernel<4, 1, 2, true, false, false, false, true>), grid, dim3(256), lds, stream, p);
+    else if (p.Nw % 4 == 0) hipLaunchKernelGGL((wino_kernel<4, 1, 2, true, false>), grid, dim3(256), lds, stream, p);
     else hipLaunchKernelGGL((wino_kernel<1, 1, 2, true, false>), grid, dim3(256), lds, stream, p);
     hipError_t e = hipGetLastError();
     if (e != hipSuccess) return e;
diff --git a/stereo-3d-reconstruction_amd/csrc/s3r_host.h b/stereo-3d-reconstruction_amd/csrc/s3r_host.h
--- a/stereo-3d-reconstruction_amd/csrc/s3r_host.h
+++ b/stereo-3d-reconstruction_amd/csrc/s3r_host.h
@@ -126,6 +126,8 @@
 int wino2_form_of(const s3r_conv_desc* d, int ntotal, int forced);
 WinoNeed wino2_need(const s3r_conv_desc* d, int form);
 double wino2_exec_flops(const s3r_conv_desc* d);
+inline bool layout_dh(int layout) { return layout == S3R_LAYOUT_WINO_DH || layout == S3R_LAYOUT_WINO_DH_CV; }
+bool cv_zero_used(const s3r_conv_desc* d);
 int cout_pad_h(int cout);
 s3r::ConvParamsH make_params_h(const s3r_conv_desc* d, const Geo& g);
 int resolve_launch_h(const s3r_conv_desc* d, s3r::ConvParamsH* p, LaunchH* L);
diff --git a/stereo-3d-reconstruction_amd/csrc/s3r_kernels.h b/stereo-3d-reconstruction_amd/csrc/s3r_kernels.h
--- a/stereo-3d-reconstruction_amd/csrc/s3r_kernels.h
+++ b/stereo-3d-reconstruction_amd/csrc/s3r_kernels.h
@@ -101,7 +101,49 @@
     const float* xd;
     int xd_mode;
     int out_mode;
-};
+    int cv;
+    FastDiv dCvSd, dCvSH;
+};
+
+#if defined(__HIPCC__)
+__host__ __device__
+#endif
+inline int cv_live_halves(int sd, int wq, int a, int edge, int wq_last = -1) {
+    const int d_min = a == 0 ? (sd == 0 ? 1 : 4 * sd - 1) : 4 * sd;
+    if (wq_last < wq) wq_last = wq;
+    const int w_max = 4 * wq_last + 4 < edge - 1 ? 4 * wq_last + 4 : edge - 1;
+    const int w_min = wq == 0 ? 0 : 4 * wq - 1;
+    return (w_max >= d_min ? 1 : 0) | (w_min + d_min < edge ? 2 : 0);
+}
+#if defined(__HIPCC__)
+__host__ __device__
+#endif
+inline void cv_zones(int sd, int nq, int& lo, int& hi) {
+    int q1 = sd - 1 < 0 ? 0 : sd - 1, q2 = nq + 1 - sd > nq ? nq : nq + 1 - sd;
+    if (q1 > nq) q1 = nq;
+    if (q1 <= q2) {
+        if (q1 == 1) q1 = 0;
+        if (nq - q2 == 1) q2 = nq;
+        lo = q1; hi = q2;
+    } else { lo = q2; hi = q1; }
+}
+#if defined(__HIPCC__)
+__device__ __forceinline__ void cv_decode(const ConvParams& p, int n, int& b, int& sd, int& sh, int& pw, int& q0, int& gw) {
+    sd = p.dCvSd.div(n);
+    int r = n - sd * (p.B * p.Nh * p.Nw);
+    const int nq = p.Nw >> 2, unit = p.B * p.Nh * 4;
+    int lo, hi;
+    cv_zones(sd, nq, lo, hi);
+    if (r < unit * lo) { q0 = 0; gw = lo; }
+    else if (r < unit * hi) { q0 = lo; gw = hi - lo; }
+    else { q0 = hi; gw = nq - hi; }
+    r -= unit * q0;
+    const int brow = (int)((unsigned)r / (unsigned)(4 * gw));
+    b = p.dCvSH.div(brow);
+    sh = brow - b * p.Nh;
+    pw = 4 * q0 + (r - brow * 4 * gw);
+}
+#endif
 
 struct TClsEntry {
     int Nd, Nh, Nw, kd, kh, kw, T, x_org, y_org, Ntotal, wg_begin, w_off;
@@ -164,6 +206,8 @@
 hipError_t launch_wino2p_input(const float* x, float* V, int B, int Cin, int Hp, int Wp, int SH, int SW, long long npad, hipStream_t s);
 hipError_t launch_pack_wino2(const float* w, float* wp, int ax, int Cin, int Cout, int CoutPad, hipStream_t s);
 int wino2_form(int ax, int cout, int ntotal, int forced);
+int wino2_cv_group(int edge, int sd, int q);
+double wino2_cv_live_share(int batch, int edge);
 int64_t wino2_slab_elems(int ax, int cout, int ntotal, int form);
 int64_t wino2_npad(int64_t ntotal);
 hipError_t launch_conv_wino2(ConvParams p, int ax, int form, bool to_v, hipStream_t stream, int* launches);
diff --git a/stereo-3d-reconstruction_amd/csrc/s3r_plan.hip b/stereo-3d-reconstruction_amd/csrc/s3r_plan.hip
--- a/stereo-3d-reconstruction_amd/csrc/s3r_plan.hip
+++ b/stereo-3d-reconstruction_amd/csrc/s3r_plan.hip
@@ -135,7 +135,7 @@
     if (d->in_halo < 0 || d->out_halo < 0 || d->in_halo > 8 || d->out_halo > 8)
         return fail(S3R_ERR_INVALID, "halo must be in [0, 8]");
     if (d->dtype != S3R_F32 && d->dtype != S3R_BF16) return fail(S3R_ERR_INVALID, "unknown dtype %d", d->dtype);
-    if ((d->in_layout != S3R_LAYOUT_PLAIN && d->in_layout != S3R_LAYOUT_WINO_H && d->in_layout != S3R_LAYOUT_WINO_DH &&
+    if ((d->in_layout != S3R_LAYOUT_PLAIN && d->in_layout != S3R_LAYOUT_WINO_H && !layout_dh(d->in_layout) &&
          d->in_layout != S3R_LAYOUT_WINO_HW && d->in_layout != S3R_LAYOUT_WINO_3D && d->in_layout != S3R_LAYOUT_DIFF) ||
         (d->out_layout != S3R_LAYOUT_PLAIN && d->out_layout != S3R_LAYOUT_WINO_HW && d->out_layout != S3R_LAYOUT_WINO_3D &&
          d->out_layout != S3R_LAYOUT_DIFF))
@@ -197,10 +197,13 @@
         if (g->in % wino_r(d) != 0) return fail(S3R_ERR_INVALID, "a Winograd-transformed input needs an edge that is a multiple of %d", wino_r(d));
         g->x_elems = (wino_r(d) + 2) * (int64_t)d->batch * d->cin * (g->nd == 3 ? g->in_p : 1) * (g->in / wino_r(d)) * g->in_p;
     }
-    if (d->in_layout == S3R_LAYOUT_WINO_DH) {
+    if (layout_dh(d->in_layout)) {
         if (d->dtype != S3R_F32 || d->op != S3R_OP_CONV || d->ndim != 3 || d->stride != 1 || d->k != 3 || d->pad != 1 || (g->in & 3) ||
             d->in_halo != 1 || d->cin % 32 != 0 || d->cout <= 1)
             return fail(S3R_ERR_INVALID, "a two-axis Winograd-transformed input serves an fp32 Conv3d k=3 s=1 p=1 over an edge %% 4 == 0, in_halo = 1");
+        if (d->in_layout == S3R_LAYOUT_WINO_DH_CV && ((d->cin & 1) || (d->cin / 2) % s3r::wino_bk() != 0))
+            return fail(S3R_ERR_INVALID, "a two-axis Winograd-transformed input with the cost volume's zero statement (S3R_LAYOUT_WINO_DH_CV) "
+                        "serves an fp32 Conv3d k=3 s=1 p=1 over an edge %% 4 == 0, in_halo = 1, with cin / 2 a multiple of %d", s3r::wino_bk());
         g->x_elems = 36 * (int64_t)d->batch * d->cin * (g->in / 4) * (g->in / 4) * g->in_p;
     }
     if (d->in_layout == S3R_LAYOUT_WINO_HW) {
@@ -336,7 +339,7 @@
 }
 bool wino2_desc_ok(const s3r_conv_desc* d) {
     return wino2_ax(d) >= 0 && d->act < S3R_ACT_SIGMOID && dil_of(d) == 1 && d->in_halo == d->pad && d->ksplit <= 1 &&
-           (d->in_layout == S3R_LAYOUT_PLAIN || (d->in_layout == S3R_LAYOUT_WINO_DH && wino2_ax(d) == 0 && d->in_size % 4 == 0) ||
+           (d->in_layout == S3R_LAYOUT_PLAIN || (layout_dh(d->in_layout) && wino2_ax(d) == 0 && d->in_size % 4 == 0) ||
             (d->in_layout == S3R_LAYOUT_WINO_HW && wino2_ax(d) == 2 && d->in_size % 4 == 0) ||
             (d->in_layout == S3R_LAYOUT_WINO_3D && wino2_ax(d) <= 1)) &&
            (d->out_layout == S3R_LAYOUT_PLAIN || (d->out_layout == S3R_LAYOUT_WINO_HW && wino2_ax(d) == 2 && d->in_size % 4 == 0) ||
@@ -346,7 +349,7 @@
     return d->algo == S3R_ALGO_DIRECT || (d->algo == S3R_ALGO_AUTO && (d->tile >= 0 || d->ksplit >= 1));
 }
 static bool two_axis_io(const s3r_conv_desc* d) {
-    if (d->in_layout == S3R_LAYOUT_WINO_DH || d->in_layout == S3R_LAYOUT_WINO_HW || d->in_layout == S3R_LAYOUT_WINO_3D ||
+    if (layout_dh(d->in_layout) || d->in_layout == S3R_LAYOUT_WINO_HW || d->in_layout == S3R_LAYOUT_WINO_3D ||
         d->out_layout == S3R_LAYOUT_WINO_HW)
         return true;
     return d->op == S3R_OP_CONV && (d->out_layout == S3R_LAYOUT_WINO_3D || d->out_layout == S3R_LAYOUT_DIFF) && wino2_ax(d) >= 0 &&
@@ -521,7 +524,7 @@
     WinoNeed w = {0, 0, 0};
     const Wino2Geo g2 = wino2_geo(d);
     if (d->batch <= 0 || g2.bmax <= 0) return w;
-    if (d->in_layout != S3R_LAYOUT_WINO_DH && d->in_layout != S3R_LAYOUT_WINO_HW && d->in_layout != S3R_LAYOUT_WINO_3D)
+    if (!layout_dh(d->in_layout) && d->in_layout != S3R_LAYOUT_WINO_HW && d->in_layout != S3R_LAYOUT_WINO_3D)
         w.v = ((g2.ax == 2 ? g2.ncls * d->cin * s3r::wino2_npad(g2.pos_sample * g2.bmax) : g2.v_sample * g2.bmax) + 255) / 256 * 256;
     for (int b0 = 0; b0 < d->batch; b0 += g2.bmax) {
         const int nb = d->batch - b0 < g2.bmax ? d->batch - b0 : g2.bmax;
@@ -535,7 +538,8 @@
 }
 double wino2_exec_flops(const s3r_conv_desc* d) {
     const Wino2Geo g2 = wino2_geo(d);
-    return 2.0 * (double)g2.pos_sample * d->batch * g2.ncls * d->cout * d->cin * g2.kw;
+    const double all = 2.0 * (double)g2.pos_sample * d->batch * g2.ncls * d->cout * d->cin * g2.kw;
+    return cv_zero_used(d) ? all * s3r::wino2_cv_live_share(d->batch < g2.bmax ? d->batch : g2.bmax, d->in_size) : all;
 }
 int cout_pad_h(int cout) { return (cout + 63) / 64 * 64; }
 
@@ -754,6 +758,9 @@
 static int handoff_mask() {
     static const int m = getenv("S3R_WINO_HANDOFF") ? atoi(getenv("S3R_WINO_HANDOFF")) : 1;
     return m == 1 ? ~0 : m;
+}
+bool cv_zero_used(const s3r_conv_desc* d) {
+    return d->in_layout == S3R_LAYOUT_WINO_DH_CV && d->out_layout == S3R_LAYOUT_PLAIN && (handoff_mask() & 64);
 }
 
 static int handoff3d(const s3r_conv_desc& a, const s3r_conv_desc& b, bool* take) {
@@ -1042,4 +1049,17 @@
     return wino_input_layout(d, &elems);
 }
 
-}
+int s3r_cv_column_group(int in_size, int depth_group, int column_quad) {
+    if (in_size < 4 || in_size % 4 != 0 || depth_group < 0 || depth_group >= in_size / 4 || column_quad < 0 || column_quad >= in_size / 4)
+        return fail(S3R_ERR_INVALID, "s3r_cv_column_group: in_size a multiple of 4, depth_group and column_quad in [0, in_size / 4)");
+    return s3r::wino2_cv_group(in_size, depth_group, column_quad);
+}
+
+int s3r_cv_zero_skip(int in_size, int depth_group, int column_quad, int depth_class) {
+    if (in_size < 4 || in_size % 4 != 0 || depth_group < 0 || depth_group >= in_size / 4 || column_quad < 0 || column_quad >= in_size / 4 ||
+        depth_class < 0 || depth_class >= 6)
+        return fail(S3R_ERR_INVALID, "s3r_cv_zero_skip: in_size a multiple of 4, depth_group and column_quad in [0, in_size / 4), depth_class in [0, 6)");
+    return 3 & ~s3r::cv_live_halves(depth_group, column_quad, depth_class, in_size);
+}
+
+}
diff --git a/stereo-3d-reconstruction_amd/modules.py b/stereo-3d-reconstruction_amd/modules.py
--- a/stereo-3d-reconstruction_amd/modules.py
+++ b/stereo-3d-reconstruction_amd/modules.py
@@ -304,7 +304,7 @@
              x2: Optional[torch.Tensor] = None, in_layout: int = 0) -> torch.Tensor:
         lib = _lib.load()
         device, batch = x.device, x.shape[0] + (x2.shape[0] if x2 is not None else 0)
-        if in_layout in (_lib.LAYOUT_WINO_H, _lib.LAYOUT_WINO_DH):
+        if in_layout in _WINO_IN_LAYOUTS:
             batch = x.shape[1]
         if batch == 0:
             n0 = len(self._layers) if upto is None else self.names.index(upto) + 1
@@ -501,11 +501,13 @@
                                                              self.max_disp, H, W, _stream_ptr(fl.device)), "cost_volume (wino2)")
         return self._planes
 
-    def forward_for(self, consumer, feat_left: torch.Tensor, feat_right: torch.Tensor):
+    def forward_for(self, consumer, feat_left: torch.Tensor, feat_right: torch.Tensor, zero_statement: bool = False):
         layout = consumer.wino_input_layout(feat_left.shape[0])
         if layout == _lib.LAYOUT_WINO_H:
             return self.forward_wino(feat_left, feat_right), layout
         if layout == _lib.LAYOUT_WINO_DH:
+            if zero_statement and feat_left.dim() == 4 and self.max_disp == feat_left.shape[2] == feat_left.shape[3]:
+                layout = _lib.LAYOUT_WINO_DH_CV
             return self.forward_wino2(feat_left, feat_right), layout
         return self.forward_padded(feat_left, feat_right), _lib.LAYOUT_PLAIN
 
@@ -533,8 +535,11 @@
         return differentiable_cost_volume(feat_left, feat_right, self.max_disp)
 
 
+_WINO_IN_LAYOUTS = (_lib.LAYOUT_WINO_H, _lib.LAYOUT_WINO_DH, _lib.LAYOUT_WINO_DH_CV)
+
+
 def _check_wino_planes(v: torch.Tensor, layout: int = _lib.LAYOUT_WINO_H) -> torch.Tensor:
-    if layout == _lib.LAYOUT_WINO_DH:
+    if layout in (_lib.LAYOUT_WINO_DH, _lib.LAYOUT_WINO_DH_CV):
         ncls, want = 36, (2 * spec.FEAT_C, spec.MAX_DISP // 4, spec.FEAT_HW // 4, spec.FEAT_HW + 2)
     else:
         ncls, want = 6, (2 * spec.FEAT_C, spec.MAX_DISP + 2, spec.FEAT_HW // 4, spec.FEAT_HW + 2)
@@ -561,7 +566,7 @@
 
     def forward_padded(self, volume_padded: torch.Tensor, halo: int = 1, in_layout: int = 0, upto: Optional[str] = None) -> torch.Tensor:
         last = upto is None or upto == self.names[-1]
-        if in_layout in (_lib.LAYOUT_WINO_H, _lib.LAYOUT_WINO_DH):
+        if in_layout in _WINO_IN_LAYOUTS:
             y = self._run(_check_wino_planes(volume_padded, in_layout), upto, in_halo=1, in_layout=in_layout)
             return y.squeeze(1) if last else y
         n = (spec.MAX_DISP + 2 * halo, spec.FEAT_HW + 2 * halo, spec.FEAT_HW + 2 * halo)
@@ -614,7 +619,7 @@
         return self._run(_check_input(volume, "volume", tail))
 
     def forward_padded(self, volume_padded: torch.Tensor, halo: int = 1, in_layout: int = 0) -> torch.Tensor:
-        if in_layout in (_lib.LAYOUT_WINO_H, _lib.LAYOUT_WINO_DH):
+        if in_layout in _WINO_IN_LAYOUTS:
             return self._run(_check_wino_planes(volume_padded, in_layout), None, in_halo=1, in_layout=in_layout)
         n = (spec.MAX_DISP + 2 * halo, spec.FEAT_HW + 2 * halo, spec.FEAT_HW + 2 * halo)
         if self.precision == "bf16":
@@ -748,7 +753,7 @@
             l, r = left[s:s + MAX_CHUNK], right[s:s + MAX_CHUNK]
             b = l.shape[0]
             feats = self.encoder.forward_pair(l, r)
-            vol, layout = self.cost_volume.forward_for(self.decoder, feats[:b], feats[b:])
+            vol, layout = self.cost_volume.forward_for(self.decoder, feats[:b], feats[b:], zero_statement=True)
             yield self.decoder.forward_padded(vol, in_layout=layout, upto=upto)
 
     @torch.no_grad()
@@ -806,7 +811,7 @@
             l, r = left[s:s + MAX_CHUNK], right[s:s + MAX_CHUNK]
             b = l.shape[0]
             feats = self.encoder.forward_pair(l, r)
-            vol, layout = self.cost_volume.forward_for(self.decoder, feats[:b], feats[b:])
+            vol, layout = self.cost_volume.forward_for(self.decoder, feats[:b], feats[b:], zero_statement=True)
             latent = self.decoder.forward_padded(vol, in_layout=layout)
             if latent.dtype != torch.float32:
                 latent = channels_last_to_f32(latent)
```

Result: no change. 8910 (median of 6 runs) (+0.9%).
